# ZikangYuan/sr_livo

Measured on AMD Instinct MI355X. Metric: sweeps/s (full ESIKF solve of a 64k-pt Livox sweep vs 1M-pt voxel map), higher is better.
Workload: dtype f64; 1 GPU; HEADLINE: stream of 4 distinct 65536-keypoint livox sweeps (own poses and priors), 978481-pt voxel map (1000000 target), max_num_residuals=2147483647, r=1, K=20; one full ESIKF solve per sweep, every sweep crosses PCIe once (uploaded on the copy stream during the solve before it: resident in HBM when its solve starts); sweeps drawn with seeds 20251309 + 100 j, keeping those that take sweep 0's 2 E; parallelism=single GPU

## Files before the change

### include/srlivo_hip_debug.h

```cpp
#ifndef SRLIVO_HIP_DEBUG_H
#define SRLIVO_HIP_DEBUG_H

#include "srlivo_hip.h"

#ifdef __cplusplus
extern "C" {
#endif

int srl_debug_set_select_mode(srl_ctx *ctx, int select_mode);

int srl_debug_radix_sort_pairs(srl_ctx *ctx, const uint32_t *keys, int n, int bits, uint32_t *keys_sorted, uint32_t *positions_sorted);

int srl_debug_color_map_rebuilds(srl_ctx *ctx, int32_t *voxel_table, int32_t *grid_table);

int srl_debug_set_frame_order_mode(srl_ctx *ctx, int mode);
int srl_debug_frame_order_used(srl_ctx *ctx, int *used);

int srl_debug_set_gather_counts(srl_ctx *ctx, int nranks, int rank, const int64_t *counts);

int srl_debug_set_ablate(srl_ctx *ctx, int bits);
int srl_debug_set_fused_reduce(srl_ctx *ctx, int enable);
int srl_debug_set_bound_culling(srl_ctx *ctx, int enable);
int srl_debug_set_pose_box(srl_ctx *ctx, int kind);
int srl_debug_set_arm_linger(srl_ctx *ctx, double host_linger_us, double kernel_linger_us);
int srl_debug_pass_stamps(srl_ctx *ctx, int enable, long long *gpu_out, long long *host_out);
int srl_debug_frame_timing(srl_ctx *ctx, int enable, double out16[16]);
int srl_debug_set_frame_epoch(srl_ctx *ctx, int frames_to_wrap);
int srl_debug_set_launch_shape(srl_ctx *ctx, int keypoints_per_wave, int waves_per_workgroup);
int srl_debug_set_search_select_mode(srl_ctx *ctx, int select_mode);
int srl_debug_heap_topk(const double *distances, int n, int K, int32_t *out_index);
int srl_debug_device_sqrt(srl_ctx *ctx, const double *in, int n, double *out);
int srl_debug_block_times(srl_ctx *ctx, double *out, int max_blocks, int *nblocks);

#ifdef __cplusplus
}
#endif
#endif
```

### sr_livo_amd/capi.py

```python
import ctypes as C
import os
import re

import numpy as np

_HERE = os.path.dirname(os.path.abspath(__file__))
LIB_PATH = os.environ.get("SRL_LIB_PATH") or os.path.join(_HERE, "libsrlivo_hip.so")
INCLUDE_DIR = os.path.join(os.path.dirname(_HERE), "include")

SRL_OK = 0
SRL_ERR_NO_DEVICE = -1
SRL_ERR_BAD_ARG = -3
SRL_ERR_UNSUPPORTED = -4
SRL_ERR_COMM = -7
SRL_ERR_NAN_PLANARITY = -8
SRL_ERR_NOT_ENOUGH_RESIDUALS = -9
SRL_COMM_ID_BYTES = 128


SRL_PEER_HANDLE_BYTES = 64


class SrlError(RuntimeError):
    def __init__(self, status, what, detail=""):
# ... 119 lines not shown
        raise SrlError(-1, "libsrlivo_hip.so not built",
                       f"(expected {LIB_PATH}; run `python -c 'import __graft_entry__ as g; g.build()'`)")
    lib = C.CDLL(LIB_PATH)
    p = C.c_void_p
    dp = C.POINTER(C.c_double)
    sig = {
        "srl_device_count": ([C.POINTER(C.c_int)], C.c_int),
        "srl_ctx_create": ([C.c_int, C.POINTER(p)], C.c_int),
        "srl_ctx_destroy": ([p], C.c_int),
        "srl_last_error": ([p], C.c_char_p),
        "srl_status_str": ([C.c_int], C.c_char_p),
        "srl_icp_opts_default": ([C.POINTER(IcpOpts)], None),
        "srl_map_upload": ([p, p, p, p, C.c_int, C.c_int], C.c_int),
        "srl_map_insert": ([p, p, C.c_int, C.c_double, C.c_int, C.c_double, C.c_int, C.POINTER(C.c_int)], C.c_int),
        "srl_map_insert_report": ([p, p, C.c_int, C.c_double, C.c_int, C.c_double, C.c_int, C.c_double, p, p, C.POINTER(C.c_int),
                                   C.POINTER(C.c_int)], C.c_int),
        "srl_map_size": ([p, C.POINTER(C.c_int64), C.POINTER(C.c_int32)], C.c_int),
        "srl_map_download": ([p, p, p, p, C.c_int], C.c_int),
        "srl_map_remove_far": ([p, dp, C.c_double, C.POINTER(C.c_int32), C.POINTER(C.c_int64)], C.c_int),
        "srl_map_probe_checksum": ([p, p, C.c_int, C.c_int, C.c_double, C.POINTER(C.c_uint64)], C.c_int),
        "srl_color_opts_default": ([C.POINTER(ColorOpts)], None),
        "srl_color_map_create": ([p, C.POINTER(ColorOpts)], C.c_int),
        "srl_color_map_destroy": ([p], C.c_int),
        "srl_color_map_insert": ([p, p, C.c_int, C.c_double, C.c_double, p, p, C.c_int, p, C.c_int, C.POINTER(ColorTotals)], C.c_int),
        "srl_color_map_size": ([p, C.POINTER(C.c_int64), C.POINTER(C.c_int32), C.POINTER(C.c_int64), C.POINTER(C.c_int64)], C.c_int),
        "srl_color_map_download": ([p, p, p, p, C.c_int, p, p, C.c_int64], C.c_int),
        "srl_color_registered_download": ([p, C.c_int64, C.c_int, p], C.c_int),
        "srl_debug_color_map_rebuilds": ([p, C.POINTER(C.c_int32), C.POINTER(C.c_int32)], C.c_int),
        "srl_color_image_upload": ([p, p, C.c_int, C.c_int, C.c_int64], C.c_int),
        "srl_color_select_opts_default": ([C.POINTER(ColorSelectOpts)], None),
        "srl_color_map_select": ([p, C.POINTER(ColorCamera), C.c_int, C.c_int, p, C.c_int, C.POINTER(ColorSelectOpts), p, C.c_int64,
                                  C.POINTER(ColorSelectTotals)], C.c_int),
        "srl_color_map_render": ([p, C.POINTER(ColorCamera), p, C.c_int, C.c_double, C.POINTER(ColorRenderTotals)], C.c_int),
        "srl_color_map_download_rgb": ([p, p, p, p, p, p, C.c_int64], C.c_int),
        "srl_color_registered_rgb": ([p, C.c_int64, C.c_int, p, p, p, p, p], C.c_int),
        "srl_sweep_upload": ([p, p, C.c_int], C.c_int),
        "srl_sweep_shard": ([p, C.POINTER(C.c_int), C.POINTER(C.c_int), C.POINTER(C.c_int)], C.c_int),
        "srl_sweep_prefetch": ([p, p, C.c_int], C.c_int),
        "srl_sweep_swap": ([p], C.c_int),
        "srl_sweep_wait": ([p], C.c_int),
        "srl_thread_pin_to_gpu_numa": ([p, C.POINTER(C.c_int)], C.c_int),
        "srl_pinned_alloc": ([C.c_size_t, C.POINTER(p)], C.c_int),
        "srl_pinned_free": ([p], C.c_int),
        "srl_host_register": ([p, C.c_size_t], C.c_int),
        "srl_host_unregister": ([p], C.c_int),
        "srl_comm_backend_info": ([C.c_char_p, C.c_int, C.POINTER(C.c_int), C.POINTER(C.c_int)], C.c_int),
        "srl_build_residuals": ([p, C.POINTER(Frame), C.POINTER(IcpOpts), C.POINTER(NormalEq)], C.c_int),
        "srl_build_residuals_overlap": ([p, C.POINTER(Frame), C.POINTER(IcpOpts), C.POINTER(NormalEq), p, p], C.c_int),
        "srl_set_taps": ([p, C.c_int], C.c_int),
        "srl_fetch_neighbors": ([p, p, p, p], C.c_int),
        "srl_fetch_residuals": ([p, p, p, p, p, p, p], C.c_int),
        "srl_search_neighbors": ([p, p, C.c_int, C.c_int, C.c_double, C.c_int, C.c_int, p, p, p], C.c_int),
        "srl_transform_points": ([p, p, C.c_int, dp, dp, dp, dp, p], C.c_int),
        "srl_frame_upload": ([p, p, C.c_int], C.c_int),
        "srl_frame_undistort": ([p, p, p, p, C.c_int, p, C.c_int, C.c_double, C.c_int, dp, dp, p, p], C.c_int),
        "srl_frame_take": ([p, p, C.c_int], C.c_int),
        "srl_frame_subsample": ([p, p, C.c_int, C.c_double, C.POINTER(C.c_int)], C.c_int),
        "srl_frame_take_subsampled": ([p, p, C.c_int, p, p, p], C.c_int),
        "srl_frame_size": ([p, C.POINTER(C.c_int)], C.c_int),
        "srl_frame_select_keypoints": ([p, dp, dp, dp, dp, C.c_double, p, C.POINTER(C.c_int)], C.c_int),
        "srl_frame_commit_report": ([p, dp, dp, dp, dp, C.c_double, C.c_int, C.c_double, C.c_int, p, p, p, C.POINTER(C.c_int),
                                     C.POINTER(C.c_int)], C.c_int),
        "srl_frame_commit": ([p, dp, dp, dp, dp, C.c_double, C.c_int, C.c_double, C.c_int, p, C.POINTER(C.c_int)], C.c_int),
        "srl_comm_unique_id": ([p], C.c_int),
        "srl_comm_init_rank": ([p, C.c_int, C.c_int, p], C.c_int),
        "srl_comm_destroy": ([p], C.c_int),
        "srl_comm_set_library": ([C.c_char_p], C.c_int),
        "srl_comm_suspend": ([p, C.c_int], C.c_int),
        "srl_comm_info": ([p, C.POINTER(C.c_int), C.POINTER(C.c_int), C.POINTER(C.c_int), C.POINTER(C.c_int), C.POINTER(C.c_int64)], C.c_int),
        "srl_comm_set_host_callbacks": ([p, C.c_int, C.c_int, ALLREDUCE_FN, ALLGATHER_FN, p], C.c_int),
        "srl_debug_set_gather_counts": ([p, C.c_int, C.c_int, C.POINTER(C.c_int64)], C.c_int),
        "srl_peer_export": ([p, p, C.POINTER(p)], C.c_int),
        "srl_peer_attach": ([p, C.c_int, C.c_int, p, C.POINTER(p)], C.c_int),
        "srl_peer_set_deadline_ms": ([p, C.c_int], C.c_int),
        "srl_peer_stats": ([p, C.POINTER(C.c_int64), C.POINTER(C.c_int)], C.c_int),
        "srl_peer_detach": ([p], C.c_int),
        "srl_shard_range": ([C.c_int, C.c_int, C.c_int, C.POINTER(C.c_int), C.POINTER(C.c_int)], None),
        "srl_shard_budget": ([C.c_int, C.POINTER(C.c_int64), C.c_int, C.c_int, C.POINTER(C.c_int64), C.POINTER(C.c_int)], None),
        "srl_get_timing": ([p, C.POINTER(Timing)], C.c_int),
        "srl_debug_block_times": ([p, p, C.c_int, C.POINTER(C.c_int)], C.c_int),
        "srl_debug_set_ablate": ([p, C.c_int], C.c_int),
        "srl_debug_set_fused_reduce": ([p, C.c_int], C.c_int),
        "srl_debug_set_bound_culling": ([p, C.c_int], C.c_int),
        "srl_debug_set_pose_box": ([p, C.c_int], C.c_int),
        "srl_debug_set_arm_linger": ([p, C.c_double, C.c_double], C.c_int),
        "srl_debug_pass_stamps": ([p, C.c_int, p, p], C.c_int),
        "srl_debug_frame_timing": ([p, C.c_int, p], C.c_int),
        "srl_debug_set_frame_epoch": ([p, C.c_int], C.c_int),
        "srl_set_armed_launch": ([p, C.c_int], C.c_int),
        "srl_disarm": ([p], C.c_int),
        "srl_solve_end": ([p], C.c_int),
        "srl_get_arm_stats": ([p, C.POINTER(C.c_uint64)], C.c_int),
        "srl_debug_set_launch_shape": ([p, C.c_int, C.c_int], C.c_int),
        "srl_debug_set_search_select_mode": ([p, C.c_int], C.c_int),
        "srl_debug_set_select_mode": ([p, C.c_int], C.c_int),
        "srl_debug_set_frame_order_mode": ([p, C.c_int], C.c_int),
        "srl_debug_radix_sort_pairs": ([p, p, C.c_int, C.c_int, p, p], C.c_int),
        "srl_debug_frame_order_used": ([p, C.POINTER(C.c_int)], C.c_int),
        "srl_debug_heap_topk": ([p, C.c_int, C.c_int, p], C.c_int),
        "srl_debug_device_sqrt": ([p, p, C.c_int, p], C.c_int),
        "srl_set_profiling": ([p, C.c_int], C.c_int),
        "srl_set_profiling_period": ([p, C.c_int], C.c_int),
        "srl_timing_mark": ([p], C.c_int),
        "srl_lio_create": ([C.c_int, C.POINTER(p)], C.c_int),
        "srl_lio_destroy": ([p], C.c_int),
        "srl_lio_ctx": ([p], p),
        "srl_lio_last_error": ([p], C.c_char_p),
        "srl_lio_set_extrinsics": ([p, dp, dp], C.c_int),
        "srl_lio_set_laser_point_cov": ([p, C.c_double], C.c_int),
        "srl_lio_last_solve_launches": ([p, C.POINTER(C.c_int)], C.c_int),
        "srl_lio_eskf_get_state": ([p, dp], C.c_int),
        "srl_lio_eskf_set_state": ([p, dp], C.c_int),
        "srl_lio_eskf_get_cov": ([p, dp], C.c_int),
        "srl_lio_eskf_set_cov": ([p, dp], C.c_int),
        "srl_lio_eskf_set_noise": ([p, C.c_double, C.c_double, C.c_double, C.c_double], C.c_int),
        "srl_lio_eskf_init_imu": ([p, dp, dp], C.c_int),
        "srl_lio_eskf_scale_init_cov": ([p], C.c_int),
        "srl_lio_eskf_predict": ([p, C.c_double, dp, dp], C.c_int),
        "srl_lio_eskf_observe": ([p, dp], C.c_int),
        "srl_lio_add_points_to_map": ([p, p, C.c_int, C.c_double, C.c_int, C.c_double, C.c_int], C.c_int),
        "srl_lio_map_size": ([p, C.POINTER(C.c_int64)], C.c_int),
        "srl_lio_remove_points_far_from_location": ([p, dp, C.c_double], C.c_int),
        "srl_lio_set_collect_points_world": ([p, C.c_int], C.c_int),
        "srl_lio_points_world": ([p, p, C.c_int, C.POINTER(C.c_int)], C.c_int),
        "srl_lio_set_device_subsample": ([p, C.c_int], C.c_int),
        "srl_lio_set_color_map_options": ([p, C.POINTER(ColorOpts)], C.c_int),
        "srl_lio_set_color_times": ([p, C.c_double, C.c_double, C.c_int], C.c_int),
        "srl_lio_add_points_to_map_at": ([p, p, C.c_int, C.c_double, C.c_int, C.c_double, C.c_int, C.c_double, C.c_int], C.c_int),
        "srl_lio_select_points_for_projection": ([p, C.POINTER(ColorCamera), C.c_int, C.c_int, C.c_double, C.c_int, C.c_int, C.c_int, p, C.c_int,
                                                  C.POINTER(C.c_int), C.POINTER(ColorSelectTotals)], C.c_int),
        "srl_lio_color_visited": ([p, C.c_int, p, C.c_int, C.POINTER(C.c_int), C.POINTER(C.c_int)], C.c_int),
        "srl_lio_color_stored": ([p, p, C.c_int, C.POINTER(C.c_int)], C.c_int),
        "srl_lio_render_points_in_recent_voxel": ([p, C.POINTER(ColorCamera), C.c_double, C.POINTER(ColorRenderTotals)], C.c_int),
        "srl_lio_probe_checksum_of_committed_frame": ([p, C.c_int, C.c_double, C.POINTER(C.c_uint64), C.POINTER(C.c_int32)], C.c_int),
        "srl_lio_resident_sweep": ([p, p, C.c_int], C.c_int),
        "srl_lio_prefetch_sweep": ([p, p, C.c_int], C.c_int),
        "srl_lio_swap_sweep": ([p], C.c_int),
        "srl_lio_prefetch_sweep_during_solve": ([p, p, C.c_int], C.c_int),
        "srl_lio_update_iekf": ([p, C.POINTER(IcpOpts), p, C.c_int, dp, dp, C.c_int, p, C.c_int,
                                 C.POINTER(C.c_int), C.POINTER(C.c_int)], C.c_int),
        "srl_lio_stream_step": ([p, C.POINTER(IcpOpts), dp, dp, C.c_int, dp, dp, C.c_int, p, C.c_int, C.POINTER(C.c_int), C.POINTER(C.c_int)], C.c_int),
        "srl_lio_update_iekf_provided": ([p, C.POINTER(IcpOpts), PROVIDER_FN, p, C.c_int, dp, dp, C.c_int, p, C.c_int,
                                          C.POINTER(C.c_int), C.POINTER(C.c_int)], C.c_int),
        "srl_lio_optimize": ([p, C.POINTER(IcpOpts), C.c_double, p, p, C.c_int, dp, dp, C.c_int, p,
                              C.POINTER(C.c_int), C.POINTER(C.c_int), C.POINTER(C.c_int)], C.c_int),
        "srl_lio_eskf_try_init": ([p, dp, dp, dp, C.c_int, C.POINTER(C.c_int)], C.c_int),
        "srl_lio_eskf_get_init_stats": ([p, dp], C.c_int),
        "srl_lio_set_initial_flag": ([p, C.c_int], C.c_int),
        "srl_lio_state_initialization": ([p, C.c_int, C.c_int, dp, dp, dp], C.c_int),
        "srl_lio_set_odometry_options": ([p, C.POINTER(OdometryOpts)], C.c_int),
        "srl_lio_run_measurement": ([p, C.c_double, p, p, p, C.c_int, p, p, C.c_int, C.c_double, C.c_double,
                                     C.POINTER(ReplayResult)], C.c_int),
        "srl_lio_last_frame": ([p, C.c_int, p, p, p, C.POINTER(C.c_int)], C.c_int),
        "srl_lio_optimize_resident": ([p, C.POINTER(IcpOpts), C.c_double, p, C.c_int, dp, dp, C.c_int, p,
                                       C.POINTER(C.c_int), C.POINTER(C.c_int), C.POINTER(C.c_int)], C.c_int),
        "srl_lio_commit_frame": ([p, dp, C.c_double, C.c_int, C.c_double, C.c_int, p, C.POINTER(C.c_int)], C.c_int),
        "srl_lio_search_neighbors": ([p, dp, C.c_int, C.c_double, C.c_int, C.c_int, p, p, C.POINTER(C.c_int)], C.c_int),
        "srl_lio_neighborhood": ([p, p, C.c_int, dp, dp, dp, dp], C.c_int),
        "srl_lio_build_plane_residuals": ([p, C.POINTER(IcpOpts), p, C.c_int, dp, dp, C.c_int, p, C.c_int,
                                           C.POINTER(C.c_int), dp, C.POINTER(C.c_int), p], C.c_int),
        "srl_grid_sampling": ([p, C.c_int, C.c_double, p, C.POINTER(C.c_int)], C.c_int),
        "srl_debug_tr1_order": ([p, C.c_int, p], C.c_int),
        "srl_debug_tr1_order_by_relation": ([p, C.c_int, p], C.c_int),
    }
    for name, (argtypes, restype) in sig.items():
        fn = getattr(lib, name)
# ... 339 lines not shown
        self._chk(self.lib.srl_sweep_wait(self.h), "srl_sweep_wait")

    def sweep_swap(self):
        self._chk(self.lib.srl_sweep_swap(self.h), "srl_sweep_swap")

    def sweep_shard(self):
        b, c, t = C.c_int(), C.c_int(), C.c_int()
        self._chk(self.lib.srl_sweep_shard(self.h, C.byref(b), C.byref(c), C.byref(t)), "srl_sweep_shard")
        return b.value, c.value, t.value

    def set_taps(self, on):
        self._chk(self.lib.srl_set_taps(self.h, int(on)), "srl_set_taps")

    def set_profiling(self, on):
        self._chk(self.lib.srl_set_profiling(self.h, int(on)), "srl_set_profiling")

    def timing_mark(self):
        self._chk(self.lib.srl_timing_mark(self.h), "srl_timing_mark")

    def set_profiling_period(self, period):
        self._chk(self.lib.srl_set_profiling_period(self.h, int(period)), "srl_set_profiling_period")

    def timing(self):
        t = Timing()
        self._chk(self.lib.srl_get_timing(self.h, C.byref(t)), "srl_get_timing")
        return t

    def _select(self, opts):
        mode = int(getattr(opts, "select_mode", 0) or 0)
        if mode != getattr(self, "_select_mode", 0):
            self._chk(self.lib.srl_debug_set_select_mode(self.h, mode), "srl_debug_set_select_mode")
            self._select_mode = mode

    def build_residuals(self, frame, opts, allow=(SRL_ERR_NAN_PLANARITY,)):
        self._select(opts)
        out = NormalEq()
        rc = self._chk(self.lib.srl_build_residuals(self.h, C.byref(frame), C.byref(opts), C.byref(out)), "srl_build_residuals", ok=allow)
        return out, rc

    def build_residuals_overlap(self, frame, opts, fn, allow=(SRL_ERR_NAN_PLANARITY,)):
        self._select(opts)
        out = NormalEq()
        cb = C.CFUNCTYPE(None, C.c_void_p)(lambda _u: fn())
        rc = self._chk(self.lib.srl_build_residuals_overlap(self.h, C.byref(frame), C.byref(opts), C.byref(out), cb, None),
                       "srl_build_residuals_overlap", ok=allow)
        return out, rc

    def pin_thread_to_gpu_numa(self):
        node = C.c_int(-1)
        rc = self.lib.srl_thread_pin_to_gpu_numa(self.h, C.byref(node))
        return node.value if rc == 0 else None

    def fetch_neighbors(self, K=20):
        _, n, _ = self.sweep_shard()
        ids = np.empty((n, K), dtype=np.int32)
        status = np.empty(n, dtype=np.uint8)
        ncand = np.empty(n, dtype=np.int32)
        self._chk(self.lib.srl_fetch_neighbors(self.h, _ptr(ids), _ptr(status), _ptr(ncand)), "srl_fetch_neighbors")
        return ids, status, ncand

    def fetch_residuals(self):
        _, n, _ = self.sweep_shard()
        normal = np.empty((n, 3)); a2d = np.empty(n); w = np.empty(n); off = np.empty(n); d = np.empty(n); J = np.empty((n, 6))
        self._chk(self.lib.srl_fetch_residuals(self.h, _ptr(normal), _ptr(a2d), _ptr(w), _ptr(off), _ptr(d), _ptr(J)), "srl_fetch_residuals")
        return dict(normal=normal, a2D=a2d, weight=w, norm_offset=off, distance=d, jacobian=J)

    def search_neighbors(self, world_xyz, nb=1, size=1.0, K=20, thr=1):
        q = _f64(world_xyz, (-1, 3))
        ids = np.empty((len(q), K), dtype=np.int32)
        xyz = np.empty((len(q), K, 3), dtype=np.float32)
        nf = np.empty(len(q), dtype=np.int32)
        self._chk(self.lib.srl_search_neighbors(self.h, _ptr(q), len(q), nb, size, K, thr, _ptr(ids), _ptr(xyz), _ptr(nf)), "srl_search_neighbors")
        return ids, xyz, nf

    def set_launch_shape(self, kpw, wpb):
        self._chk(self.lib.srl_debug_set_launch_shape(self.h, int(kpw), int(wpb)), "srl_debug_set_launch_shape")

    def set_fused_reduce(self, on):
        self._chk(self.lib.srl_debug_set_fused_reduce(self.h, 1 if on else 0), "srl_debug_set_fused_reduce")

    def set_bound_culling(self, on):
        self._chk(self.lib.srl_debug_set_bound_culling(self.h, 1 if on else 0), "srl_debug_set_bound_culling")

    def set_search_select_mode(self, mode):
        self._chk(self.lib.srl_debug_set_search_select_mode(self.h, int(mode)), "srl_debug_set_search_select_mode")

    def set_armed_launch(self, on):
        mode = int(on) if on in (0, 1, 2) and not isinstance(on, bool) else (1 if on else 0)
        self._chk(self.lib.srl_set_armed_launch(self.h, mode), "srl_set_armed_launch")

    def solve_end(self):
        self._chk(self.lib.srl_solve_end(self.h), "srl_solve_end")

    def disarm(self):
        self._chk(self.lib.srl_disarm(self.h), "srl_disarm")

    def arm_stats(self):
        out = (C.c_uint64 * 4)()
        self._chk(self.lib.srl_get_arm_stats(self.h, out), "srl_get_arm_stats")
        return dict(zip(("armed", "fired", "cancelled", "expired"), (int(v) for v in out)))

    def set_pose_box(self, kind):
        self._chk(self.lib.srl_debug_set_pose_box(self.h, int(kind)), "srl_debug_set_pose_box")

    FRAME_STAGES = ("upload", "select_group", "select_download", "select_host_order", "select_gather", "commit_transform", "commit_download",
                    "insert_sort", "insert_segments", "insert_lookup_create", "insert_replay")

    def set_frame_epoch(self, frames_to_wrap):
        self._chk(self.lib.srl_debug_set_frame_epoch(self.h, int(frames_to_wrap)), "srl_debug_set_frame_epoch")

    def frame_timing(self, enable=True):
        out = np.zeros(16)
        self._chk(self.lib.srl_debug_frame_timing(self.h, 1 if enable else 0, _ptr(out)), "srl_debug_frame_timing")
        return dict(zip(self.FRAME_STAGES, (float(v) for v in out)))

    def pass_stamps(self, enable=True, read=True):
        g = np.zeros((64, 32), dtype=np.int64); h = np.zeros((64, 4), dtype=np.int64)
        self._chk(self.lib.srl_debug_pass_stamps(self.h, 1 if enable else 0, _ptr(g) if read else None, _ptr(h) if read else None), "srl_debug_pass_stamps")
        return g, h

    def set_arm_linger(self, host_linger_us=150.0, kernel_linger_us=300.0):
        self._chk(self.lib.srl_debug_set_arm_linger(self.h, float(host_linger_us), float(kernel_linger_us)), "srl_debug_set_arm_linger")

    def device_sqrt(self, x):
        x = _f64(x).ravel()
        out = np.empty_like(x)
        self._chk(self.lib.srl_debug_device_sqrt(self.h, _ptr(x), len(x), _ptr(out)), "srl_debug_device_sqrt")
        return out

    def transform_points(self, raw_xyz, q, t, R_il=None, t_il=None):
        r = _f64(raw_xyz, (-1, 3))
        out = np.empty_like(r)
        R_il = _f64(np.eye(3) if R_il is None else R_il).ravel()
        t_il = _f64(np.zeros(3) if t_il is None else t_il)
        self._chk(self.lib.srl_transform_points(self.h, _ptr(r), len(r), _dptr(_f64(q)), _dptr(_f64(t)), _dptr(R_il), _dptr(t_il), _ptr(out)), "srl_transform_points")
        return out

    def frame_upload(self, raw_xyz):
        r = _f64(raw_xyz, (-1, 3))
        self._chk(self.lib.srl_frame_upload(self.h, _ptr(r), len(r)), "srl_frame_upload")

    def frame_undistort(self, raw_xyz, relative_time_ms, imu_states, time_frame_begin, mode, R_il=None, t_il=None, imu_point_in=None,
                        want_outputs=True):
        r = _f64(raw_xyz, (-1, 3)); rel = _f64(relative_time_ms)
        st = _f64(imu_states, (-1, 17))
        R_il = _f64(np.eye(3) if R_il is None else R_il).ravel()
        t_il = _f64(np.zeros(3) if t_il is None else t_il)
        pin = None if imu_point_in is None else _f64(imu_point_in, (-1, 3))
        imu = np.empty_like(r) if want_outputs else None
        out = np.empty_like(r) if want_outputs else None
        self._chk(self.lib.srl_frame_undistort(self.h, _ptr(r), _ptr(rel), None if pin is None else _ptr(pin), len(r), _ptr(st), len(st),
                                               float(time_frame_begin), int(mode), _dptr(R_il), _dptr(t_il), _ptr(imu), _ptr(out)),
                  "srl_frame_undistort")
        return imu, out

    def frame_take(self, index):
        idx = np.ascontiguousarray(index, dtype=np.int32)
        self._chk(self.lib.srl_frame_take(self.h, _ptr(idx), len(idx)), "srl_frame_take")

    def frame_subsample(self, order, sample_size):
        o = np.ascontiguousarray(order, dtype=np.int32)
        m = C.c_int()
        self._chk(self.lib.srl_frame_subsample(self.h, _ptr(o), len(o), float(sample_size), C.byref(m)), "srl_frame_subsample")
        self._kept = m.value
        return m.value

# ... 494 lines not shown
```

### sr_livo_amd/csrc/srl_capi.cpp

```cpp
#include "../../include/srlivo_hip.h"
#include "../../include/srlivo_hip_debug.h"
#include "host/srl_la.h"
#include "srl_device.h"
#include "srl_hash.h"
#include "srl_heap.h"

#include <hip/hip_runtime.h>
#include <sched.h>

#include <algorithm>
#include <atomic>
#include <chrono>
#include <climits>
#include <cstdio>
#include <cstdlib>
#include <cstring>
#include <mutex>
#include <string>
#include <vector>

struct SrlMapState;
int srl_map_insert_device(struct srl_ctx *ctx, const double *world_xyz, int n, double voxel_size, int cap,
                          double min_distance_points, int min_num_points, int *num_added);

#include "srl_ctx.h"
int srl_map_insert_report_device(srl_ctx *ctx, const double *world_xyz, int n, double voxel_size, int cap, double min_distance_points, int min_num_points,
                                 double ref_z, uint8_t *outcome, srl_cloud_point *cloud, int *num_cloud, int *num_added);

namespace {

unsigned next_pow2(unsigned v) { unsigned p = 1; while (p < v) p <<= 1; return p; }
inline long long steady_ns() { return std::chrono::duration_cast<std::chrono::nanoseconds>(std::chrono::steady_clock::now().time_since_epoch()).count(); }

constexpr int SRL_MAX_DEVICES = 64;
std::atomic<int> g_live_ctx[SRL_MAX_DEVICES];
inline int live_contexts(int device) { return (device >= 0 && device < SRL_MAX_DEVICES) ? g_live_ctx[device].load(std::memory_order_relaxed) : 1; }

int ensure_work(srl_ctx *ctx, int n) {
    if (n <= ctx->work_cap) return SRL_OK;
    const int cap = std::max(n, 1024);
    const int nblocks = std::max((cap + SRL_KPB - 1) / SRL_KPB, 1024 + 8);
    int rc;
    if ((rc = ensure(ctx, ctx->d_rec, (size_t)cap * 8))) return rc;
    if ((rc = ensure(ctx, ctx->d_status, (size_t)cap))) return rc;
    if ((rc = ensure(ctx, ctx->d_bound, (size_t)cap * 4))) return rc;
    ctx->bound_n = 0;
    if ((rc = ensure(ctx, ctx->d_partials, (size_t)nblocks * SRL_PART_STRIDE))) return rc;
    if ((rc = ensure(ctx, ctx->d_binfo, (size_t)nblocks))) return rc;
    ctx->work_cap = cap;
    ctx->block_cap = nblocks;
    return SRL_OK;
}

bool srl_is_pinned(const void *p) {
    hipPointerAttribute_t attr;
    if (hipPointerGetAttributes(&attr, p) != hipSuccess) { (void)hipGetLastError(); return false; }
    return attr.type == hipMemoryTypeHost;
}

int srl_ring_init(srl_ctx *ctx) {
    if (ctx->h_ring) return SRL_OK;
    HIPCHK(ctx, hipHostMalloc((void **)&ctx->h_ring, (size_t)srl_ctx::RING_SLOTS * srl_ctx::RING_SLOT_BYTES, hipHostMallocDefault));
    for (int i = 0; i < srl_ctx::RING_SLOTS; i++) { HIPCHK(ctx, hipEventCreateWithFlags(&ctx->ring_ev[i], hipEventDisableTiming)); ctx->ring_busy[i] = false; }
    return SRL_OK;
}

int ensure_taps(srl_ctx *ctx, int n, int K) {
    if (n <= ctx->tap_cap && K <= ctx->tap_K) return SRL_OK;
    const int cap = std::max(n, ctx->tap_cap), kk = std::max(K, ctx->tap_K);
    int rc;
    if ((rc = ensure(ctx, ctx->d_tap_ids, (size_t)cap * kk))) return rc;
    if ((rc = ensure(ctx, ctx->d_tap_ncand, (size_t)cap))) return rc;
    if ((rc = ensure(ctx, ctx->d_tap_normal, (size_t)cap * 3))) return rc;
    if ((rc = ensure(ctx, ctx->d_tap_a2d, (size_t)cap))) return rc;
    if ((rc = ensure(ctx, ctx->d_tap_offset, (size_t)cap))) return rc;
    ctx->tap_cap = cap;
    ctx->tap_K = kk;
    return SRL_OK;
}

}

int srl_ctx_ensure_work(srl_ctx *ctx, int n) { return ensure_work(ctx, n); }
bool srl_ctx_is_pinned(const void *p) { return srl_is_pinned(p); }

int srl_ctx_grow_map(srl_ctx *ctx, unsigned need_slabs, unsigned need_slots);

extern "C" {

int srl_device_count(int *count) {
    int c = 0;
    if (hipGetDeviceCount(&c) != hipSuccess) { if (count) *count = 0; return SRL_ERR_NO_DEVICE; }
    if (count) *count = c;
    return SRL_OK;
}

const char *srl_status_str(int s) {
    switch (s) {
        case SRL_OK: return "ok";
        case SRL_ERR_NO_DEVICE: return "no HIP device (the product has no CPU fallback)";
        case SRL_ERR_HIP: return "HIP runtime error";
        case SRL_ERR_BAD_ARG: return "bad argument";
        case SRL_ERR_UNSUPPORTED: return "option outside the supported envelope";
        case SRL_ERR_NO_MAP: return "no map uploaded";
        case SRL_ERR_NO_SWEEP: return "no sweep uploaded";
        case SRL_ERR_COMM: return "RCCL error";
        case SRL_ERR_NAN_PLANARITY: return "NaN planarity (optimize.cpp:348-350 throws)";
        case SRL_ERR_NOT_ENOUGH_RESIDUALS: return "not enough residuals (optimize.cpp:110)";
        default: return "unknown status";
    }
}

void srl_icp_opts_default(srl_icp_opts *o) {
    o->threshold_voxel_occupancy = 1;
    o->init_num_frames = 20;
    o->size_voxel_map = 1.0;
    o->num_iters_icp = 5;
    o->min_number_neighbors = 20;
    o->voxel_neighborhood = 1;
    o->power_planarity = 2.0;
    o->max_number_neighbors = 20;
    o->max_dist_to_plane_icp = 0.3;
    o->threshold_orientation_norm = 0.1;
    o->threshold_translation_norm = 0.01;
    o->max_num_residuals = 600;
    o->weight_alpha = 0.9;
    o->weight_neighborhood = 0.1;
}

int srl_ctx_create(int device, srl_ctx **out) {
    if (!out) return SRL_ERR_BAD_ARG;
    *out = nullptr;
    int count = 0;
    if (hipGetDeviceCount(&count) != hipSuccess || count <= 0 || device < 0 || device >= count) return SRL_ERR_NO_DEVICE;
    if (hipSetDevice(device) != hipSuccess) return SRL_ERR_NO_DEVICE;
    srl_ctx *ctx = new srl_ctx();
    ctx->device = device;
    { int cu = 0; if (hipDeviceGetAttribute(&cu, hipDeviceAttributeMultiprocessorCount, device) == hipSuccess && cu > 0) ctx->num_cu = cu; }
    if (hipStreamCreateWithFlags(&ctx->stream, hipStreamNonBlocking) != hipSuccess) { delete ctx; return SRL_ERR_NO_DEVICE; }
    if (hipMalloc((void **)&ctx->d_out, sizeof(SrlDevOut)) != hipSuccess ||
        hipHostMalloc((void **)&ctx->h_out, sizeof(SrlDevOut)) != hipSuccess ||
        hipMalloc((void **)&ctx->d_count, sizeof(long long)) != hipSuccess ||
        hipHostMalloc((void **)&ctx->h_count, sizeof(long long)) != hipSuccess) {
        delete ctx;
        return SRL_ERR_HIP;
    }
    {
        const size_t row_bytes = (size_t)(SRL_FUSED_MAX_BLOCKS + SRL_FUSED_MAX_GROUPS) * SRL_ROW_GRANULES * 8;
        if (hipMalloc((void **)&ctx->d_granules, row_bytes) != hipSuccess || hipMemset(ctx->d_granules, 0, row_bytes) != hipSuccess) { delete ctx; return SRL_ERR_HIP; }
    }
    if (hipHostMalloc((void **)&ctx->h_mail, sizeof(SrlMailbox), hipHostMallocCoherent | hipHostMallocMapped) != hipSuccess) {
        delete ctx;
        return SRL_ERR_HIP;
    }
    std::memset(ctx->h_mail, 0, sizeof(SrlMailbox));
    for (int i = 0; i < 4; i++) hipEventCreate(&ctx->ev[i]);
    if (device < SRL_MAX_DEVICES) g_live_ctx[device].fetch_add(1, std::memory_order_relaxed);
    ctx->counted = true;
    *out = ctx;
    return SRL_OK;
}

int srl_ctx_destroy(srl_ctx *ctx) {
    if (!ctx) return SRL_OK;
    hipSetDevice(ctx->device);
    if (ctx->counted && ctx->device < SRL_MAX_DEVICES) g_live_ctx[ctx->device].fetch_sub(1, std::memory_order_relaxed);
    if (ctx->armed) srl_ctx_disarm(ctx);
    if (ctx->stream) hipStreamSynchronize(ctx->stream);
    if (ctx->copy_stream) hipStreamSynchronize(ctx->copy_stream);
    if (ctx->color) srl_color_map_destroy(ctx);
    if (ctx->pose_box_pinned) hipHostFree(ctx->pose_box_pinned);
    if (ctx->pose_box_dev) hipFree(ctx->pose_box_dev);
    if (ctx->d_pose_relay) hipFree(ctx->d_pose_relay);
    if (ctx->comm && srl_rccl()) srl_rccl()->CommDestroy(ctx->comm);
    if (ctx->parked_comm && srl_rccl()) srl_rccl()->CommDestroy(ctx->parked_comm);
    if (ctx->d_sub_kept) hipFree(ctx->d_sub_kept);
    if (ctx->d_sub_seen) hipFree(ctx->d_sub_seen);
    void *bufs[] = {ctx->d_corr_in, ctx->d_corr_rel, ctx->d_corr_imu, ctx->d_corr_raw, ctx->d_corr_seg, ctx->d_frame_raw, ctx->d_frame_world, ctx->d_table, ctx->d_slabs, ctx->d_raw, ctx->d_rec, ctx->d_status, ctx->d_partials, ctx->d_binfo,
                    ctx->d_out, ctx->d_count, ctx->d_bound, ctx->d_granules, ctx->d_rec_granules, ctx->d_raw_next, ctx->d_stage_next, ctx->d_stage_cur, ctx->d_tap_ids, ctx->d_tap_ncand, ctx->d_tap_normal, ctx->d_tap_a2d,
                    ctx->d_tap_offset, ctx->d_gather, ctx->d_peer, ctx->d_mail};
    for (int r = 0; r < SRL_MAX_PEERS; r++) if (ctx->peer_mapped[r]) hipIpcCloseMemHandle(ctx->peer_mapped[r]);
    if (ctx->d_inbox) hipFree(ctx->d_inbox);
    for (void *b : bufs) if (b) hipFree(b);
    if (ctx->h_out) hipHostFree(ctx->h_out);
    if (ctx->h_count) hipHostFree(ctx->h_count);
    if (ctx->h_mail) hipHostFree(ctx->h_mail);
    if (ctx->h_arm_stamps) hipHostFree(ctx->h_arm_stamps);
    if (ctx->h_scratch) hipHostFree(ctx->h_scratch);
    if (ctx->h_frame_x) hipHostFree(ctx->h_frame_x);
    for (SrlEpochTable *t : {&ctx->sel_table, &ctx->ins_table}) { if (t->keyw) hipFree(t->keyw); if (t->minw) hipFree(t->minw); }
    if (ctx->d_frame_sync) hipFree(ctx->d_frame_sync);
    if (ctx->d_tr1_sched) hipFree(ctx->d_tr1_sched);
    if (ctx->h_insert_cnt) hipHostFree(ctx->h_insert_cnt);
    if (ctx->ev_insert) hipEventDestroy(ctx->ev_insert);
    if (ctx->ev_world) hipEventDestroy(ctx->ev_world);
    if (ctx->ev_frame_read) hipEventDestroy(ctx->ev_frame_read);
    if (ctx->h_ring) { hipHostFree(ctx->h_ring); for (int i = 0; i < srl_ctx::RING_SLOTS; i++) if (ctx->ring_ev[i]) hipEventDestroy(ctx->ring_ev[i]); }
    for (auto &b : ctx->pool_free) hipFree(b.p);
    ctx->pool_free.clear();
    for (int i = 0; i < 4; i++) if (ctx->ev[i]) hipEventDestroy(ctx->ev[i]);
    for (int i = 0; i < srl_ctx::PROF_RING; i++) for (int k = 0; k < 2; k++) if (ctx->ring[i][k]) hipEventDestroy(ctx->ring[i][k]);
    for (int sl = 0; sl < 2; sl++) for (int k = 0; k < 2; k++) if (ctx->up_ev[sl][k]) hipEventDestroy(ctx->up_ev[sl][k]);
    if (ctx->upload_ev) hipEventDestroy(ctx->upload_ev);
    if (ctx->copy_stream) { hipStreamSynchronize(ctx->copy_stream); hipStreamDestroy(ctx->copy_stream); }
    if (ctx->prefix_stream) { hipStreamSynchronize(ctx->prefix_stream); hipStreamDestroy(ctx->prefix_stream); }
    if (ctx->stream) hipStreamDestroy(ctx->stream);
    delete ctx;
    return SRL_OK;
}

const char *srl_last_error(const srl_ctx *ctx) { return ctx ? ctx->err.c_str() : "null context"; }

int srl_map_upload(srl_ctx *ctx, const int16_t *keys_xyz, const int32_t *counts, const float *xyz, int V, int cap) {
    if (!ctx || V < 0 || (V > 0 && (!keys_xyz || !counts || !xyz))) return SRL_ERR_BAD_ARG;
    SRL_DISARM(ctx);
    if (cap != SRL_VOXEL_CAP) { ctx->err = "max_num_points_in_voxel must be 20"; return SRL_ERR_UNSUPPORTED; }
    HIPCHK(ctx, hipSetDevice(ctx->device));
    { const int rcs = srl_map_settle(ctx); if (rcs) return rcs; }
    ctx->bound_n = 0;
    const unsigned slab_cap = std::max<unsigned>(1024u, (unsigned)V + (unsigned)V / 2u + 4096u);
    if (slab_cap > SRL_MAX_SLABS) { ctx->err = "map too large: slab byte offsets are 32-bit (16.7 M voxels)"; return SRL_ERR_UNSUPPORTED; }
    const unsigned table_cap = next_pow2(std::max<unsigned>(2048u, SRL_TABLE_FACTOR * slab_cap));
    std::vector<SrlSlab> slabs((size_t)V);
    std::vector<SrlMapSlot> table((size_t)table_cap);
    for (auto &s : table) { s.key = SRL_EMPTY_KEY; s.slab = 0; s.count = 0; }
    long long npts = 0;
    const unsigned mask = table_cap - 1;
    for (int v = 0; v < V; v++) {
        SrlSlab &s = slabs[v];
        std::memset(&s, 0, sizeof s);
        const int c = counts[v];
        if (c < 0 || c > cap) { ctx->err = "voxel count out of range"; return SRL_ERR_BAD_ARG; }
        for (int i = 0; i < c; i++)
            for (int d = 0; d < 3; d++) s.xyz[i][d] = xyz[((size_t)v * cap + i) * 3 + d];
        s.count = (unsigned)c;
        s.key = srl_pack_key(keys_xyz[3 * v], keys_xyz[3 * v + 1], keys_xyz[3 * v + 2]);
        npts += c;
        unsigned h = srl_hash_key(s.key) & mask;
        while (table[h].key != SRL_EMPTY_KEY) {
            if (table[h].key == s.key) { ctx->err = "duplicate voxel key in upload"; return SRL_ERR_BAD_ARG; }
            h = (h + 1) & mask;
        }
        table[h].key = s.key;
        table[h].slab = (unsigned)v;
        table[h].count = (unsigned)c;
    }
    if (ctx->d_slabs) { HIPCHK(ctx, hipFree(ctx->d_slabs)); ctx->d_slabs = nullptr; }
    if (ctx->d_table) { HIPCHK(ctx, hipFree(ctx->d_table)); ctx->d_table = nullptr; }
    HIPCHK(ctx, hipMalloc((void **)&ctx->d_slabs, ((size_t)slab_cap + 1) * SRL_SLAB_BYTES));
    HIPCHK(ctx, hipMemsetD32Async((hipDeviceptr_t)(ctx->d_slabs + (size_t)slab_cap * SRL_SLAB_BYTES), 0x7f800000, SRL_SLAB_BYTES / 4, ctx->stream));
    HIPCHK(ctx, hipMalloc((void **)&ctx->d_table, (size_t)table_cap * sizeof(SrlMapSlot)));
    HIPCHK(ctx, hipMemsetAsync(ctx->d_slabs, 0, (size_t)slab_cap * SRL_SLAB_BYTES, ctx->stream));
    if (V > 0) HIPCHK(ctx, hipMemcpyAsync(ctx->d_slabs, slabs.data(), (size_t)V * SRL_SLAB_BYTES, hipMemcpyHostToDevice, ctx->stream));
    HIPCHK(ctx, hipMemcpyAsync(ctx->d_table, table.data(), (size_t)table_cap * sizeof(SrlMapSlot), hipMemcpyHostToDevice, ctx->stream));
    HIPCHK(ctx, hipStreamSynchronize(ctx->stream));
    ctx->slab_cap = slab_cap;
    ctx->table_cap = table_cap;
    ctx->num_voxels = V;
    ctx->num_points = npts;
    return SRL_OK;
}

// ... 567 lines not shown
    if (ctx->force_kpw) {
        p.kpw = ctx->force_kpw;
        const bool only16 = p.kpw != 4 && p.kpw != 8 && p.kpw != 16;
        p.wpb = ((ctx->force_wpb == 16 || only16) && srl_assoc_lds_bytes(p.K, p.nb, p.kpw, 16) <= SRL_LDS_LIMIT) ? 16 : 4;
        if (only16 && p.wpb != 16) p.kpw = 4;
    }
    if (ctx->ablate != 0 && srl_assoc_lds_bytes(p.K, p.nb, 16, 16) <= SRL_LDS_LIMIT) { p.kpw = 16; p.wpb = 16; }
    p.kpb = p.kpw * p.wpb;
    p.nblocks = (n_eff + p.kpb - 1) / p.kpb;

    p.cut = cut_possible(ctx, o);
    p.transport = pass_transport(ctx);
    p.dbg_gather = ctx->dbg_gather;
    const bool fusable = !ctx->taps && ctx->ablate == 0 && o->max_num_residuals > 0 && ctx->fuse_reduce && !ctx->dbg_gather;
    p.fuse_cut = fusable && p.cut && p.transport == Transport::single && p.wpb == 16 && p.kpb <= SRL_FUSED_CUT_MAX_KPB && p.nblocks <= 512;
    p.fused = p.fuse_cut || (fusable && !p.cut && p.wpb == 16 && p.nblocks <= SRL_FUSED_MAX_BLOCKS);
    p.tagged_mail = p.fused && p.transport != Transport::rccl;
    p.mailbox = p.transport != Transport::rccl && (p.transport == Transport::single || p.fused);
    const bool fast_sel = ctx->select_mode == 0 || ctx->select_mode == 4;
    p.arm_ok = ctx->arm_mode != 0 && p.fused && fast_sel && ctx->profiling != 1 && (p.transport != Transport::host_callback || ctx->cb_ar);
    return SRL_OK;
}

static void prepare_assoc_args(srl_ctx *ctx, const srl_frame *f, const srl_icp_opts *o, int n_eff, const PassPlan &p, SrlAssocArgs &a) {
    std::memset(&a, 0, sizeof a);
    a.raw_x = ctx->d_raw;
    a.raw_y = ctx->d_raw + ctx->sweep_cap;
    a.raw_z = ctx->d_raw + 2 * (size_t)ctx->sweep_cap;
    a.n = n_eff;
    a.aos = (n_eff > ctx->soa_valid_n) ? ctx->d_stage_cur : nullptr;
    a.table = ctx->d_table;
    a.table_mask = ctx->table_cap - 1;
    a.slabs = ctx->d_slabs;
    a.inf_off = ctx->slab_cap * (unsigned)SRL_SLAB_BYTES;
    a.write_rec = ((ctx->taps || p.cut) && !p.fuse_cut) ? 1 : 0;
    {
        const srl::Quat q(f->q[0], f->q[1], f->q[2], f->q[3]);
        const srl::Mat3 Rn = q.normalized().toRotationMatrix();
        const srl::Mat3 R = q.toRotationMatrix();
        std::memcpy(a.Rn, Rn.a, sizeof a.Rn);
        std::memcpy(a.R, R.a, sizeof a.R);
    }
    std::memcpy(a.t, f->t, sizeof a.t);
    std::memcpy(a.t_last, f->t_last, sizeof a.t_last);
    std::memcpy(a.R_il, f->R_il, sizeof a.R_il);
    std::memcpy(a.t_il, f->t_il, sizeof a.t_il);
    a.size_voxel = o->size_voxel_map;
    a.max_dist = o->max_dist_to_plane_icp;
    {
        double lw = std::abs(o->weight_alpha), ln = std::abs(o->weight_neighborhood);
        const double sum = lw + ln;
        lw /= sum;
        ln /= sum;
        a.lambda_w = lw;
        a.lambda_n = ln;
    }
    a.power_planarity = o->power_planarity;
    a.nbr_scale = o->max_dist_to_plane_icp * o->min_number_neighbors;
    a.K = p.K;
    a.min_nb = o->min_number_neighbors;
    a.thr_cap = p.thr;
    a.select_mode = ctx->select_mode;
    a.ablate = ctx->ablate;
    a.stamps = ctx->h_arm_stamps;
    a.rec = ctx->d_rec;
    a.status = ctx->d_status;
    a.partials = ctx->d_partials;
    a.binfo = ctx->d_binfo;
    if (ctx->taps) {
        a.tap_ids = ctx->d_tap_ids;
        a.tap_ncand = ctx->d_tap_ncand;
        a.tap_normal = ctx->d_tap_normal;
        a.tap_a2d = ctx->d_tap_a2d;
        a.tap_offset = ctx->d_tap_offset;
    }
    {
        float sv = (float)o->size_voxel_map;
        int sv_bits; std::memcpy(&sv_bits, &sv, 4);
        const int sig[4] = {p.K, p.nb, p.thr, sv_bits};
        if (std::memcmp(sig, ctx->bound_sig, sizeof sig) != 0) { ctx->bound_n = 0; std::memcpy(ctx->bound_sig, sig, sizeof sig); }
        a.bound_out = ctx->d_bound;
        a.bound_in = ctx->bound_mode != 0 ? ctx->d_bound : nullptr;
        a.bound_use = a.bound_in ? std::min(ctx->bound_n, n_eff) : 0;
    }
    if (p.fused) {
        a.granules = ctx->d_granules;
        a.mailbox = p.transport == Transport::rccl ? ctx->d_mail : ctx->h_mail;
        a.mail_tagged = p.tagged_mail ? 1 : 0;
    }
    if (p.fuse_cut) {
        a.rec_granules = ctx->d_rec_granules;
        a.cut_max = o->max_num_residuals;
    }
}

static int grow_pass_buffers(srl_ctx *ctx, const PassPlan &p) {
    int rc;
    ctx->taps_valid = false;
    if (ctx->taps) {
        if ((rc = ensure_taps(ctx, ctx->n, p.K))) return rc;
        if (ctx->n > 0) {
            HIPCHK(ctx, hipMemsetAsync(ctx->d_tap_ids, 0xFF, (size_t)ctx->n * p.K * sizeof(int), ctx->stream));
            HIPCHK(ctx, hipMemsetAsync(ctx->d_tap_normal, 0, (size_t)ctx->n * 3 * sizeof(double), ctx->stream));
            HIPCHK(ctx, hipMemsetAsync(ctx->d_tap_a2d, 0, (size_t)ctx->n * sizeof(double), ctx->stream));
            HIPCHK(ctx, hipMemsetAsync(ctx->d_tap_offset, 0, (size_t)ctx->n * sizeof(double), ctx->stream));
        }
    }
    ctx->last_nblocks = p.nblocks;
    if (p.nblocks > ctx->block_cap) {
        if ((rc = ensure(ctx, ctx->d_partials, (size_t)p.nblocks * SRL_PART_STRIDE))) return rc;
        if ((rc = ensure(ctx, ctx->d_binfo, (size_t)p.nblocks))) return rc;
        ctx->block_cap = p.nblocks;
    }
    if (ctx->profiling == 2 && ctx->ring_head - ctx->ring_tail >= (unsigned)srl_ctx::PROF_RING && (rc = drain_ring(ctx, true))) return rc;
    if (p.fused && p.transport == Transport::rccl && !ctx->d_mail && (rc = ensure(ctx, ctx->d_mail, 1))) return rc;
    const size_t need = (size_t)p.nblocks * p.kpb * 16;
    if (p.fuse_cut && need > ctx->rec_granule_cap) {
        if ((rc = ensure(ctx, ctx->d_rec_granules, need))) return rc;
        HIPCHK(ctx, hipMemsetAsync(ctx->d_rec_granules, 0, need * sizeof(unsigned long long), ctx->stream));
        ctx->rec_granule_cap = need;
    }
    return SRL_OK;
}

struct ExchangeTag { unsigned long long seq; unsigned epoch; int slot; };
static ExchangeTag exchange_tag(unsigned long long seq) {
    if ((unsigned)seq == 0u) ++seq;
    return {seq, (unsigned)seq, (int)(seq & 1ull)};
}
static ExchangeTag next_exchange(srl_ctx *ctx) {
    const ExchangeTag t = exchange_tag(ctx->peer_seq + 1);
    ctx->peer_seq = t.seq;
    return t;
}

static SrlAssocArgs arm_signature(const SrlAssocArgs &src) {
    SrlAssocArgs sg = src;
    std::memset(sg.Rn, 0, sizeof sg.Rn); std::memset(sg.R, 0, sizeof sg.R); std::memset(sg.t, 0, sizeof sg.t);
    std::memset(sg.t_last, 0, sizeof sg.t_last);
    sg.pose_box = nullptr; sg.pose_relay = nullptr; sg.pose_relayed = 0; sg.pose_epoch = 0; sg.arm_linger_ticks = 0;
    sg.raw_x = sg.raw_y = sg.raw_z = nullptr; sg.alt_x = sg.alt_y = sg.alt_z = nullptr; sg.n = 0; sg.aos = nullptr; sg.alt_aos = nullptr;
    sg.bound_use = 0;
    return sg;
}

static int fire_or_cancel(srl_ctx *ctx, const PassPlan &p, SrlAssocArgs &a, unsigned long long &seq_now, bool &fired) {
    fired = false;
    bool needs_tail = false;
    if (ctx->tail_pending) {
        if (hipEventQuery(ctx->up_ev[ctx->cur_slot][1]) == hipSuccess) { ctx->tail_pending = false; ctx->cur_prefix_n = ctx->n; }
        else needs_tail = a.n > ctx->cur_prefix_n;
        (void)hipGetLastError();
    }
    if (!ctx->armed) return SRL_OK;
    const SrlAssocArgs sg = arm_signature(a);
    const double age_us = (double)(steady_ns() - ctx->armed_at_ns) * 1e-3;
    const bool on_raw = a.raw_x == ctx->armed_raw && ctx->sweep_cap == ctx->armed_raw_cap && a.aos == nullptr;
    const bool on_alt = !on_raw && ctx->armed_alt != nullptr && a.raw_x == ctx->armed_alt && ctx->sweep_cap == ctx->armed_alt_cap &&
                        a.aos != nullptr && a.aos == ctx->armed_alt_aos;
    if (p.arm_ok && !needs_tail && age_us < ctx->arm_host_linger_us && p.nb == ctx->armed_nb && p.kpw == ctx->armed_kpw &&
        p.nblocks <= ctx->armed_nblocks && (on_raw || on_alt) && std::memcmp(&sg, &ctx->armed_sig, sizeof sg) == 0) {
        pose_box_write(ctx, a.Rn, a.R, a.t, (unsigned)seq_now, SRL_ARM_GO | (on_alt ? SRL_ARM_ALT : 0u), (unsigned)a.n, a.t_last);
        ctx->armed = false;
        ctx->armed_ring = -1;
        ctx->arm_stats[1]++;
        ctx->cur_measured = ctx->armed_measured;
        ctx->cur_gen = ctx->armed_gen;
        fired = true;
        return SRL_OK;
    }
    if (const int rc = srl_ctx_disarm(ctx)) return rc;
    seq_now = ++ctx->seq;
    if (p.fused) a.seq = seq_now;
    return SRL_OK;
}

static int prof_role(const srl_ctx *ctx) {
    if (ctx->prof_period <= 1) return 2;
    const unsigned long long r = ctx->prof_count % (unsigned long long)ctx->prof_period;
    return r == 1 ? 2 : (r == 0 ? 1 : 0);
}

static int launch_assoc(srl_ctx *ctx, const PassPlan &p, const SrlAssocArgs &args, bool armed) {
    if (!armed && ctx->tail_pending) {
        HIPCHK(ctx, hipStreamWaitEvent(ctx->stream, ctx->up_ev[ctx->cur_slot][1], 0));
        ctx->tail_pending = false; ctx->cur_prefix_n = ctx->n;
    }
    const bool prof = ctx->profiling == 1, prof_light = ctx->profiling == 2;
    const int role = prof_light ? prof_role(ctx) : 0;
    int prev = -1;
    if (armed && role != 0) {
        int rc;
        if (ctx->ring_head - ctx->ring_tail >= (unsigned)srl_ctx::PROF_RING - 2 && (rc = drain_ring(ctx, true))) return rc;
        if (ctx->ring_head != 0 && !ctx->ring_void[(ctx->ring_head - 1) % srl_ctx::PROF_RING] && ctx->ring_last_count == (long long)ctx->prof_count - 1)
            prev = (int)((ctx->ring_head - 1) % srl_ctx::PROF_RING);
    }
    const unsigned slot = ctx->ring_head % srl_ctx::PROF_RING;
    if (prof) HIPCHK(ctx, hipEventRecord(ctx->ev[0], ctx->stream));
    if (role == 2 && prev < 0) HIPCHK(ctx, hipEventRecord(ctx->ring[slot][0], ctx->stream));
    HIPCHK(ctx, srl_launch_assoc(args, p.nb, p.kpw, p.wpb, ctx->stream));
    if (prof) HIPCHK(ctx, hipEventRecord(ctx->ev[1], ctx->stream));
    if (role != 0) {
        HIPCHK(ctx, hipEventRecord(ctx->ring[slot][1], ctx->stream));
        ctx->ring_prev[slot] = prev; ctx->ring_marker[slot] = role == 1; ctx->ring_void[slot] = false; ctx->ring_gen[slot] = ctx->timing_gen;
        ctx->ring_last_count = (long long)ctx->prof_count;
        ctx->ring_head++;
    }
    if (prof_light) ctx->prof_count++;
    const bool measured = !prof_light || role == 2;
    if (armed) { ctx->armed_ring = role != 0 ? (int)slot : -1; ctx->armed_measured = measured; ctx->armed_gen = ctx->timing_gen; }
    else { ctx->cur_measured = measured; ctx->cur_gen = ctx->timing_gen; }
    return SRL_OK;
}

static bool arm_wanted(const srl_ctx *ctx) {
    return ctx->arm_mode == 2 ||
           (live_contexts(ctx->device) <= 1 && !ctx->peer_shares_device && !ctx->comm_shares_device &&
            (ctx->next_n >= 0 || ctx->expected_passes == 0 || ctx->passes_in_solve + 1 < ctx->expected_passes));
}

static int arm_next(srl_ctx *ctx, const PassPlan &p, const SrlAssocArgs &a) {
    int rc;
    if ((rc = ensure_pose_box(ctx))) return rc;
    SrlAssocArgs nx = a;
    nx.seq = ctx->seq + 1;
    nx.bound_use = a.bound_in ? a.n : 0;
    const bool has_alt = ctx->d_raw_next != nullptr && ctx->next_cap > 0 && ctx->d_stage_next != nullptr;
    nx.aos = nullptr;
    nx.alt_aos = has_alt ? ctx->d_stage_next : nullptr;
    nx.alt_x = has_alt ? ctx->d_raw_next : nullptr;
    nx.alt_y = has_alt ? ctx->d_raw_next + ctx->next_cap : nullptr;
    nx.alt_z = has_alt ? ctx->d_raw_next + 2 * (size_t)ctx->next_cap : nullptr;
    if (p.transport == Transport::peer) {
        const ExchangeTag t = exchange_tag(ctx->peer_seq + 1);
        nx.peer_epoch = t.epoch;
        nx.peer_slot = t.slot;
    }
    nx.pose_box = ctx->h_pose_box;
    nx.pose_relay = ctx->d_pose_relay;
    nx.pose_relayed = ctx->pose_box_kind == 1 ? 0 : 1;
    nx.pose_epoch = (unsigned)nx.seq;
    nx.arm_linger_ticks = ctx->arm_linger_ticks;
    if ((rc = launch_assoc(ctx, p, nx, true))) return rc;
    ctx->armed_sig = arm_signature(nx);
    ctx->armed_nb = p.nb; ctx->armed_kpw = p.kpw; ctx->armed_nblocks = p.nblocks;
    ctx->armed_raw = nx.raw_x; ctx->armed_raw_cap = ctx->sweep_cap;
    ctx->armed_alt = nx.alt_x; ctx->armed_alt_cap = has_alt ? ctx->next_cap : 0; ctx->armed_alt_aos = nx.alt_aos;
    ctx->armed_at_ns = steady_ns();
    ctx->armed = true;
    ctx->arm_stats[0]++;
    return SRL_OK;
}

static int reduce_unfused(srl_ctx *ctx, const PassPlan &p, const srl_icp_opts *o, int n_eff, unsigned long long seq) {
    int64_t budget = o->max_num_residuals;
    int mode = 0;
    const long long *gather = nullptr;
    if (p.transport == Transport::single || !p.cut) {
        srl_shard_budget(o->max_num_residuals, nullptr, ctx->nranks, ctx->rank, &budget, &mode);
    } else {
        HIPCHK(ctx, srl_launch_count(ctx->d_binfo, p.nblocks, o->max_num_residuals <= 0 ? 1 : 0, ctx->d_count, ctx->stream));
        if (p.transport == Transport::peer) {
            const ExchangeTag t = next_exchange(ctx);
            HIPCHK(ctx, srl_launch_peer_counts(ctx->d_peer, t.epoch, t.slot, ctx->d_count, ctx->d_gather, ctx->stream));
            gather = ctx->d_gather;
        } else if (p.transport == Transport::rccl) {
            NCCLCHK(ctx, AllGather(ctx->d_count, ctx->d_gather, 1, ncclInt64, ctx->comm, ctx->stream));
            gather = ctx->d_gather;
        } else if (p.dbg_gather) {
            gather = ctx->d_gather;
        } else {
            HIPCHK(ctx, hipMemcpyAsync(ctx->h_count, ctx->d_count, sizeof(long long), hipMemcpyDeviceToHost, ctx->stream));
            HIPCHK(ctx, hipStreamSynchronize(ctx->stream));
            if (!ctx->cb_ag) { ctx->err = "nranks > 1 without communicator"; return SRL_ERR_COMM; }
            int64_t mine = *ctx->h_count;
            std::vector<int64_t> all64((size_t)ctx->nranks, 0);
            if (ctx->cb_ag(&mine, all64.data(), ctx->cb_user) != 0) { ctx->err = "allgather callback failed"; return SRL_ERR_COMM; }
            srl_shard_budget(o->max_num_residuals, all64.data(), ctx->nranks, ctx->rank, &budget, &mode);
        }
    }
    SrlReduceArgs ra;
    ra.rec = ctx->d_rec;
    ra.status = ctx->d_status;
    ra.partials = ctx->d_partials;
    ra.binfo = ctx->d_binfo;
    ra.n = n_eff;
    ra.kpb = p.kpb;
    ra.nblocks = p.nblocks;
    ra.max_res = budget;
    ra.gather = gather;
    ra.rank = ctx->rank;
    ra.max_num_residuals = o->max_num_residuals;
    ra.out = ctx->d_out;
    ra.mailbox = p.mailbox ? ctx->h_mail : nullptr;
    ra.seq = seq;
    HIPCHK(ctx, srl_launch_reduce(ra, mode, ctx->stream));
    if (p.transport == Transport::peer) {
        const ExchangeTag t = next_exchange(ctx);
        HIPCHK(ctx, srl_launch_peer_rows(ctx->d_peer, t.epoch, t.slot, ctx->d_out, ctx->h_mail, seq, gather, ctx->stream));
    }
    return SRL_OK;
}

static int host_allreduce(srl_ctx *ctx, SrlDevOut *out) {
    if (!ctx->cb_ar) { ctx->err = "nranks > 1 without communicator"; return SRL_ERR_COMM; }
    if (ctx->cb_ar(reinterpret_cast<double *>(out), SRL_REDUCED_DOUBLES, ctx->cb_user) != 0) { ctx->err = "allreduce callback failed"; return SRL_ERR_COMM; }
    return SRL_OK;
}

// ... 14 lines not shown
            ctx->arm_stats[3]++;
            ctx->err = "armed launch expired";
            return SRL_INTERNAL_ARM_EXPIRED;
        }
        if ((++spins & 0xFFFFF) == 0) {
            const hipError_t qe = hipStreamQuery(ctx->stream);
            if (qe != hipSuccess && qe != hipErrorNotReady) { ctx->err = std::string("reduce kernel: ") + hipGetErrorString(qe); return SRL_ERR_HIP; }
            if (qe == hipSuccess && !mail_arrived(ctx, p.tagged_mail, seq)) {
                const unsigned long long *gran = ctx->h_mail->g;
                char dbg[256];
                int bad = -1; unsigned bad_tag = 0;
                if (p.tagged_mail) for (int i = 0; i < 2 * OUT_WORDS; i++) if ((unsigned)(gran[i] >> 32) != (unsigned)seq) { bad = i; bad_tag = (unsigned)(gran[i] >> 32); break; }
                std::snprintf(dbg, sizeof dbg, "reduce kernel finished without publishing (seq %llu, tagged %d, fired %d, fused %d, blocks %d, first stale granule %d tag %u, plain seq %llu)",
                              seq, (int)p.tagged_mail, (int)fired, (int)p.fused, p.nblocks, bad, bad_tag, (unsigned long long)ctx->h_mail->seq);
                ctx->err = dbg;
                return SRL_ERR_HIP;
            }
        }
    }
    if (p.tagged_mail) {
        const unsigned long long *gran = ctx->h_mail->g;
        unsigned long long *w = reinterpret_cast<unsigned long long *>(ctx->h_out);
        for (int i = 0; i < OUT_WORDS; i++)
            w[i] = (__atomic_load_n(&gran[2 * i], __ATOMIC_RELAXED) & 0xFFFFFFFFull) | (__atomic_load_n(&gran[2 * i + 1], __ATOMIC_RELAXED) << 32);
    } else {
        std::memcpy(ctx->h_out, &ctx->h_mail->out, sizeof(SrlDevOut));
    }
    return SRL_OK;
}

static int wait_result(srl_ctx *ctx, const PassPlan &p, unsigned long long seq, bool fired, long long &last_visited_local) {
    const bool copied = p.transport == Transport::host_callback && !p.fused;
    int rc;
    if (copied) {
        HIPCHK(ctx, hipMemcpyAsync(ctx->h_out, ctx->d_out, sizeof(SrlDevOut), hipMemcpyDeviceToHost, ctx->stream));
        HIPCHK(ctx, hipStreamSynchronize(ctx->stream));
    } else if ((rc = read_mailbox(ctx, p, seq, fired))) {
        return rc;
    }
    last_visited_local = ctx->h_out->last_visited;
    if (p.transport == Transport::host_callback && (rc = host_allreduce(ctx, ctx->h_out))) return rc;
    if (copied) {
        if (ctx->h_out->d_timeout > 0.5) { ctx->err = "fused final reduction timed out on another rank"; return SRL_INTERNAL_FUSED_TIMEOUT; }
        return SRL_OK;
    }
    if (ctx->h_out->pad == SRL_PEER_TIMEOUT_MARK) {
        ctx->err = "direct peer exchange: a rank's row has not arrived yet";
        return SRL_INTERNAL_PEER_TIMEOUT;
    }
    if (ctx->h_out->pad != 0 || ctx->h_out->d_timeout > 0.5) {
        ctx->err = "fused final reduction timed out waiting for a workgroup's row";
        if (fired && p.transport == Transport::rccl) ctx->arm_stats[3]++;
        return SRL_INTERNAL_FUSED_TIMEOUT;
    }
    return SRL_OK;
}

static int finish_pass(srl_ctx *ctx, const PassPlan &p, const srl_icp_opts *o, const SrlAssocArgs &a, int n_eff, long long last_visited_local,
                       unsigned long long seq, bool fired, srl_normal_eq *out) {
    const SrlDevOut &r = *ctx->h_out;
    const long long visited_total = (long long)(r.d_visited + 0.5);
    if (p.fused && !p.fuse_cut) {
        const long long expect = ctx->nranks > 1 ? (long long)ctx->total_n : (long long)n_eff;
        if (visited_total != expect) {
            char buf[256];
            std::snprintf(buf, sizeof buf, "fused pass visited %lld of %lld keypoints (fired %d, seq %llu; residuals %.0f, time-out flag %.0f, marker %lld)", visited_total, expect,
                          (int)fired, seq, r.d_num_res, r.d_timeout, (long long)r.pad);
            ctx->err = buf;
            return SRL_ERR_HIP;
        }
    }
    std::memcpy(out->HtH, r.HtH, sizeof out->HtH);
    std::memcpy(out->Hth, r.Hth, sizeof out->Hth);
    out->loss_sum = r.loss;
    out->num_residuals = (int32_t)(r.d_num_res + 0.5);
    out->success = out->num_residuals >= o->min_number_neighbors ? 1 : 0;
    out->sum_candidates = (int64_t)(r.d_sum_pk + 0.5);
    out->last_visited = visited_total - 1;
    out->nan_error = r.d_nan > 0.5 ? 1 : 0;
    out->num_fallback = (int32_t)(r.d_fallback + 0.5);

    if (a.aos != nullptr && n_eff > ctx->soa_valid_n) ctx->soa_valid_n = n_eff;
    ctx->bound_n = n_eff;
    ctx->last_K = p.K;
    ctx->last_nb = p.nb;
    ctx->last_visited_local = last_visited_local;
    ctx->taps_valid = ctx->taps;
    return SRL_OK;
}

struct PassClock { std::chrono::steady_clock::time_point entry, prep, launched, enq, res; };

static long long clock_ns(std::chrono::steady_clock::time_point t) {
    return std::chrono::duration_cast<std::chrono::nanoseconds>(t.time_since_epoch()).count();
}

static int account_pass(srl_ctx *ctx, const PassPlan &p, int n_eff, const PassClock &c) {
    using us = std::chrono::duration<double, std::micro>;
    using ms = std::chrono::duration<double, std::milli>;
    const bool prof = ctx->profiling == 1, prof_light = ctx->profiling == 2;
    if (prof) {
        HIPCHK(ctx, hipEventSynchronize(ctx->ev[3]));
        hipEventElapsedTime(&ctx->timing.assoc_ms, ctx->ev[0], ctx->ev[1]);
        hipEventElapsedTime(&ctx->timing.reduce_ms, ctx->ev[1], ctx->ev[2]);
        hipEventElapsedTime(&ctx->timing.total_ms, ctx->ev[0], ctx->ev[3]);
        ctx->timing.calls += 1;
        ctx->timing.sum_assoc_ms += ctx->timing.assoc_ms;
        ctx->timing.sum_reduce_ms += ctx->timing.reduce_ms;
        ctx->timing.sum_total_ms += ctx->timing.total_ms;
        ctx->timing.sum_keypoints += n_eff;
        const auto t_end = std::chrono::steady_clock::now();
        ctx->timing.sum_host_launch_us += us(c.enq - c.entry).count();
        ctx->timing.sum_host_wait_us += us(c.res - c.enq).count();
        ctx->timing.sum_host_total_us += us(t_end - c.entry).count();
    }
    const double sum_pk = ctx->h_out->d_sum_pk;
    const long long side = 2 * p.nb + 1;
    const long long per_kp = 24 + 12 * side * side * side;
    const double pk_share = (ctx->nranks > 1 && ctx->total_n > 0) ? sum_pk * ((double)ctx->n / (double)ctx->total_n) : sum_pk;
    ctx->timing.algorithmic_bytes = per_kp * (long long)n_eff + (long long)(12.0 * pk_share);
    if (prof || (prof_light && ctx->cur_measured && ctx->cur_gen == ctx->timing_gen)) {
        ctx->timing.sum_algorithmic_bytes += ctx->timing.algorithmic_bytes; ctx->timing.sum_keypoints += prof_light ? n_eff : 0; ctx->timing.sum_passes += 1;
    }
    if (ctx->profiling == 3) {
        ctx->timing.calls += 1;
        ctx->timing.sum_host_launch_us += us(c.launched - c.prep).count();
        ctx->timing.sum_host_wait_us += us(c.res - c.enq).count();
        ctx->timing.sum_host_total_us += us(std::chrono::steady_clock::now() - c.entry).count();
        ctx->timing.sum_assoc_ms += ms(c.prep - c.entry).count();
        ctx->timing.sum_reduce_ms += ms(c.enq - c.launched).count();
    }
    return SRL_OK;
}

static int build_residuals_pass(srl_ctx *ctx, const srl_frame *f, const srl_icp_opts *o, srl_normal_eq *out, int n_eff) {
    PassClock clk{std::chrono::steady_clock::now()};
    HIPCHK(ctx, hipSetDevice(ctx->device));
    PassPlan p;
    int rc;
    if ((rc = plan_pass(ctx, f, o, n_eff, p))) return rc;
    if ((rc = grow_pass_buffers(ctx, p))) return rc;
    SrlAssocArgs a;
    prepare_assoc_args(ctx, f, o, n_eff, p, a);
    unsigned long long seq_now = ++ctx->seq;
    if (p.transport == Transport::peer && ctx->peer_failed) {
        ctx->err = "direct peer exchange: this session has failed (a rank's row never arrived); srl_peer_detach, srl_peer_export and srl_peer_attach on every rank start a new one";
        return SRL_ERR_COMM;
    }
    if (p.fused) a.seq = seq_now;
    if (p.fused && p.transport == Transport::peer) {
        const ExchangeTag t = next_exchange(ctx);
        a.peer = ctx->d_peer; a.peer_epoch = t.epoch; a.peer_slot = t.slot;
    }
    bool fired = false;
    if ((rc = fire_or_cancel(ctx, p, a, seq_now, fired))) return rc;
    clk.prep = std::chrono::steady_clock::now();
    if (!fired && (rc = launch_assoc(ctx, p, a, false))) return rc;
    clk.launched = std::chrono::steady_clock::now();
    long long *stamps = ctx->h_arm_stamps ? ctx->arm_host_stamps[seq_now & 63ull] : nullptr;
    if (stamps) { stamps[0] = clock_ns(clk.entry); stamps[1] = clock_ns(clk.launched); stamps[3] = fired ? 1 : 0; }
    const bool arm = p.arm_ok && arm_wanted(ctx);
    if (arm && p.transport != Transport::rccl && (rc = arm_next(ctx, p, a))) return rc;
    if (!p.fused && (rc = reduce_unfused(ctx, p, o, n_eff, seq_now))) return rc;
    if (ctx->profiling == 1) HIPCHK(ctx, hipEventRecord(ctx->ev[2], ctx->stream));
    clk.enq = std::chrono::steady_clock::now();
    if (ctx->overlap_fn) {
// ... 53 lines not shown
        if (distance) distance[k] = rec[(size_t)k * 8 + 6];
        if (weight) weight[k] = rec[(size_t)k * 8 + 7];
    }
    return SRL_OK;
}

int srl_search_neighbors(srl_ctx *ctx, const double *world_xyz, int n, int nb_voxels_visited, double size_voxel_map,
                         int max_num_neighbors, int threshold_voxel_capacity, int32_t *ids, float *nb_xyz,
                         int32_t *num_found) {
    if (!ctx || n < 0 || (n > 0 && (!world_xyz || !ids || !num_found))) return SRL_ERR_BAD_ARG;
    SRL_DISARM(ctx);
    if (!ctx->d_table) return SRL_ERR_NO_MAP;
    if (nb_voxels_visited < 1 || nb_voxels_visited > 2) { ctx->err = "nb_voxels_visited must be 1 or 2"; return SRL_ERR_UNSUPPORTED; }
    if (max_num_neighbors < 1 || max_num_neighbors > SRL_MAX_NEIGHBORS) { ctx->err = "max_num_neighbors must be in [1,32]"; return SRL_ERR_UNSUPPORTED; }
    if (n == 0) return SRL_OK;
    HIPCHK(ctx, hipSetDevice(ctx->device));
    const int K = max_num_neighbors;
    DevBuf b_q, b_ids, b_nf, b_xyz;
    HIPCHK(ctx, b_q.alloc(ctx, (size_t)n * 3 * sizeof(double)));
    HIPCHK(ctx, b_ids.alloc(ctx, (size_t)n * K * sizeof(int)));
    HIPCHK(ctx, b_nf.alloc(ctx, (size_t)n * sizeof(int)));
    if (nb_xyz) HIPCHK(ctx, b_xyz.alloc(ctx, (size_t)n * K * 3 * sizeof(float)));
    double *d_q = b_q.as<double>();
    int *d_ids = b_ids.as<int>(), *d_nf = b_nf.as<int>();
    float *d_xyz = nb_xyz ? b_xyz.as<float>() : nullptr;
    HIPCHK(ctx, hipMemcpyAsync(d_q, world_xyz, (size_t)n * 3 * sizeof(double), hipMemcpyHostToDevice, ctx->stream));
    HIPCHK(ctx, hipMemsetAsync(d_ids, 0xFF, (size_t)n * K * sizeof(int), ctx->stream));
    if (d_xyz) HIPCHK(ctx, hipMemsetAsync(d_xyz, 0, (size_t)n * K * 3 * sizeof(float), ctx->stream));
    SrlSearchArgs a;
    a.q = d_q; a.n = n; a.table = ctx->d_table; a.table_mask = ctx->table_cap - 1; a.slabs = ctx->d_slabs;
    a.size_voxel = size_voxel_map; a.K = K; a.thr_cap = threshold_voxel_capacity; a.select_mode = ctx->search_select_mode;
    a.ids = d_ids; a.nb_xyz = d_xyz; a.num_found = d_nf;
    HIPCHK(ctx, srl_launch_search(a, nb_voxels_visited, ctx->stream));
    HIPCHK(ctx, hipMemcpyAsync(ids, d_ids, (size_t)n * K * sizeof(int), hipMemcpyDeviceToHost, ctx->stream));
    HIPCHK(ctx, hipMemcpyAsync(num_found, d_nf, (size_t)n * sizeof(int), hipMemcpyDeviceToHost, ctx->stream));
    if (nb_xyz) HIPCHK(ctx, hipMemcpyAsync(nb_xyz, d_xyz, (size_t)n * K * 3 * sizeof(float), hipMemcpyDeviceToHost, ctx->stream));
    HIPCHK(ctx, hipStreamSynchronize(ctx->stream));
    return SRL_OK;
}

int srl_transform_points(srl_ctx *ctx, const double *raw_xyz, int n, const double q[4], const double t[3],
                         const double R_il[9], const double t_il[3], double *out_xyz) {
    if (!ctx || n < 0 || (n > 0 && (!raw_xyz || !out_xyz)) || !q || !t || !R_il || !t_il) return SRL_ERR_BAD_ARG;
    SRL_DISARM(ctx);
    if (n == 0) return SRL_OK;
    HIPCHK(ctx, hipSetDevice(ctx->device));
    DevBuf b_in, b_o;
    HIPCHK(ctx, b_in.alloc(ctx, (size_t)n * 3 * sizeof(double)));
    HIPCHK(ctx, b_o.alloc(ctx, (size_t)n * 3 * sizeof(double)));
    double *d_in = b_in.as<double>(), *d_o = b_o.as<double>();
    HIPCHK(ctx, hipMemcpyAsync(d_in, raw_xyz, (size_t)n * 3 * sizeof(double), hipMemcpyHostToDevice, ctx->stream));
    SrlXform X;
    const srl::Mat3 R = srl::Quat(q[0], q[1], q[2], q[3]).toRotationMatrix();
    std::memcpy(X.R, R.a, sizeof X.R);
    std::memcpy(X.t, t, sizeof X.t);
    std::memcpy(X.R_il, R_il, sizeof X.R_il);
    std::memcpy(X.t_il, t_il, sizeof X.t_il);
    HIPCHK(ctx, srl_launch_transform(d_in, n, X, d_o, ctx->stream));
    HIPCHK(ctx, hipMemcpyAsync(out_xyz, d_o, (size_t)n * 3 * sizeof(double), hipMemcpyDeviceToHost, ctx->stream));
    HIPCHK(ctx, hipStreamSynchronize(ctx->stream));
    return SRL_OK;
}

int srl_debug_set_ablate(srl_ctx *ctx, int bits) {
    if (!ctx) return SRL_ERR_BAD_ARG;
    SRL_DISARM(ctx);
    ctx->ablate = bits;
    return SRL_OK;
}
int srl_debug_set_launch_shape(srl_ctx *ctx, int keypoints_per_wave, int waves_per_workgroup) {
    if (!ctx) return SRL_ERR_BAD_ARG;
    SRL_DISARM(ctx);
    if (keypoints_per_wave != 0 && keypoints_per_wave != 2 && keypoints_per_wave != 3 && keypoints_per_wave != 6 && keypoints_per_wave != 12 && keypoints_per_wave != 4 && keypoints_per_wave != 8 && keypoints_per_wave != 16) return SRL_ERR_BAD_ARG;
    if (waves_per_workgroup != 0 && waves_per_workgroup != 4 && waves_per_workgroup != 16) return SRL_ERR_BAD_ARG;
    ctx->force_kpw = keypoints_per_wave;
    ctx->force_wpb = waves_per_workgroup;
    return SRL_OK;
}
int srl_debug_set_bound_culling(srl_ctx *ctx, int enable) {
    if (!ctx) return SRL_ERR_BAD_ARG;
    SRL_DISARM(ctx);
    ctx->bound_mode = enable ? 1 : 0;
    ctx->bound_n = 0;
    return SRL_OK;
}
int srl_debug_set_fused_reduce(srl_ctx *ctx, int enable) {
    if (!ctx) return SRL_ERR_BAD_ARG;
    SRL_DISARM(ctx);
    ctx->fuse_reduce = enable != 0;
    return SRL_OK;
}
int srl_debug_set_select_mode(srl_ctx *ctx, int select_mode) {
    if (!ctx || select_mode < 0 || select_mode > 5) return SRL_ERR_BAD_ARG;
    SRL_DISARM(ctx);
    ctx->select_mode = select_mode;
    return SRL_OK;
}
int srl_debug_set_frame_order_mode(srl_ctx *ctx, int mode) {
    if (!ctx || mode < 0 || mode > 1) return SRL_ERR_BAD_ARG;
    ctx->frame_order_mode = mode;
    return SRL_OK;
}
int srl_debug_frame_order_used(srl_ctx *ctx, int *used) {
    if (!ctx || !used) return SRL_ERR_BAD_ARG;
    *used = ctx->frame_order_used;
    return SRL_OK;
}
int srl_debug_set_search_select_mode(srl_ctx *ctx, int select_mode) {
    if (!ctx || select_mode < 0 || select_mode > 5) return SRL_ERR_BAD_ARG;
    ctx->search_select_mode = select_mode;
    return SRL_OK;
}
int srl_debug_heap_topk(const double *distances, int n, int K, int32_t *out_index) {
    if (n < 0 || K < 1 || K > SRL_MAX_NEIGHBORS || (n > 0 && !distances) || !out_index) return SRL_ERR_BAD_ARG;
    double hd[SRL_MAX_NEIGHBORS];
    int he[SRL_MAX_NEIGHBORS];
    int size = 0;
    for (int i = 0; i < n; i++) size = srl_heap_offer(hd, he, size, K, distances[i], i);
    int out[SRL_MAX_NEIGHBORS];
    srl_heap_drain(hd, he, size, out);
    for (int i = 0; i < size; i++) out_index[i] = out[i];
    return size;
}
int srl_debug_device_sqrt(srl_ctx *ctx, const double *in, int n, double *out) {
    if (!ctx || n < 0 || (n > 0 && (!in || !out))) return SRL_ERR_BAD_ARG;
    SRL_DISARM(ctx);
    if (n == 0) return SRL_OK;
    HIPCHK(ctx, hipSetDevice(ctx->device));
    DevBuf b;
    HIPCHK(ctx, b.alloc(ctx, (size_t)n * sizeof(double)));
    HIPCHK(ctx, hipMemcpyAsync(b.as<double>(), in, (size_t)n * sizeof(double), hipMemcpyHostToDevice, ctx->stream));
    HIPCHK(ctx, srl_launch_sqrt(b.as<double>(), n, ctx->stream));
    HIPCHK(ctx, hipMemcpyAsync(out, b.as<double>(), (size_t)n * sizeof(double), hipMemcpyDeviceToHost, ctx->stream));
    HIPCHK(ctx, hipStreamSynchronize(ctx->stream));
    return SRL_OK;
}

void srl_shard_range(int n, int nranks, int rank, int *begin, int *count) {
    const long long b = (long long)rank * n / nranks;
    const long long e = (long long)(rank + 1) * n / nranks;
    if (begin) *begin = (int)b;
    if (count) *count = (int)(e - b);
}

void srl_shard_budget(int max_num_residuals, const int64_t *accepted_per_rank, int nranks, int rank,
                      int64_t *budget, int *mode) {
    (void)nranks;
    int64_t b = max_num_residuals;
    int m = 0;
    if (max_num_residuals <= 0) {
        int64_t prior = 0;
        for (int r = 0; r < rank; r++) prior += accepted_per_rank ? accepted_per_rank[r] : (int64_t)1;
        m = (prior > 0) ? 2 : 1;
    } else {
        int64_t prior = 0;
        for (int r = 0; r < rank; r++) prior += accepted_per_rank ? accepted_per_rank[r] : 0;
        b = (int64_t)max_num_residuals - prior;
        if (b <= 0) m = 2;
    }
    if (budget) *budget = b;
    if (mode) *mode = m;
}

int srl_build_residuals(srl_ctx *ctx, const srl_frame *f, const srl_icp_opts *o, srl_normal_eq *out) {
    if (!ctx || !f || !o || !out) return SRL_ERR_BAD_ARG;
    if (!ctx->d_table) return SRL_ERR_NO_MAP;
// ... 331 lines not shown
```

### sr_livo_amd/csrc/srl_ctx.h

```cpp
#pragma once
#include "../../include/srlivo_hip.h"
#include "srl_device.h"
#include "host/tr1_relation.h"

#include <hip/hip_runtime.h>
#include "srl_rccl.h"

#include <string>
#include <vector>

struct SrlEpochTable {
    unsigned long long *keyw = nullptr;
    unsigned long long *minw = nullptr;
    unsigned cap = 0;
    unsigned epoch16 = 0;
    unsigned counter32 = 0;
};

#define SRL_PEER_POISON_WORD SRL_PEER_INBOX_GRANULES
#define SRL_PEER_DEVICE_WORD (SRL_PEER_INBOX_GRANULES + 1)
#define SRL_PEER_INBOX_ALLOC_GRANULES (SRL_PEER_INBOX_GRANULES + 8)

struct srl_ctx {
    int device = 0;
    bool counted = false;
    hipStream_t stream = nullptr;
    std::string err;

    SrlMapSlot *d_table = nullptr;
    unsigned table_cap = 0;
    unsigned char *d_slabs = nullptr;
    unsigned slab_cap = 0;
    int num_voxels = 0;
    long long num_points = 0;

    double *d_raw = nullptr;
    int sweep_cap = 0;
    int n = 0;
    int shard_begin = 0;
    int total_n = 0;
    bool sweep_loaded = false;
    int search_select_mode = 0;
    int select_mode = 0;
    int ablate = 0;
    void (*overlap_fn)(void *) = nullptr;
    void *overlap_user = nullptr;

    double *d_raw_next = nullptr;
    double *d_stage_next = nullptr;
    double *d_stage_cur = nullptr;
    int soa_valid_n = 0;
    int next_cap = 0, stage_next_cap = 0, stage_cur_cap = 0;
    int next_n = -1, next_begin = 0, next_total = 0;
    hipStream_t copy_stream = nullptr;
    hipStream_t prefix_stream = nullptr;
    int num_cu = 256;
    hipEvent_t next_ready = nullptr;
    hipEvent_t up_ev[2][2] = {};
    bool up_one_dma[2] = {true, true};
    int next_slot = 0;
    int next_prefix_n = 0;
    int prefix_hint = 0;
    float *d_bound = nullptr;
    int bound_n = 0;
    int bound_sig[4] = {0, 0, 0, 0};
    int bound_mode = 1;
    bool tail_pending = false;
    int cur_slot = 0, cur_prefix_n = 0;

    double *d_frame_raw = nullptr;
    double *d_frame_world = nullptr;
    int frame_cap = 0;
    int frame_n = -1;
    int frame_world_n = -1;
    bool frame_world_seen = false;
    struct SrlColorMap *color = nullptr;
    double *d_corr_in = nullptr, *d_corr_rel = nullptr, *d_corr_imu = nullptr, *d_corr_raw = nullptr;
    int *d_corr_seg = nullptr;
    int corr_cap = 0;
    int corr_n = -1;
    int *d_sub_kept = nullptr;
    unsigned *d_sub_seen = nullptr;
    int sub_cap = 0;
    int sub_n = -1;
    unsigned sub_seen_tag = 0;

    bool frame_timing = false;
    double frame_stage_us[16] = {};
    long long frame_stage_last_ns = 0;

    hipEvent_t upload_ev = nullptr;
    bool upload_pending = false;

    static constexpr int RING_SLOTS = 4;
    static constexpr int RING_SLOT_BYTES = 256 * 1024;
    char *h_ring = nullptr;
    hipEvent_t ring_ev[RING_SLOTS] = {};
    bool ring_busy[RING_SLOTS] = {};
    unsigned ring_next = 0;

    char *h_scratch = nullptr;
    size_t h_scratch_bytes = 0;
    char *h_frame_x = nullptr;
    size_t h_frame_x_bytes = 0;
    unsigned *d_frame_sync = nullptr;
    unsigned frame_tag = 0;
    SrlTr1Sched *d_tr1_sched = nullptr;
    int tr1_steps = -1;
    unsigned tr1_first[SRL_TR1_MAX_STEPS] = {0}, tr1_nb[SRL_TR1_MAX_STEPS + 1] = {0};
    int frame_order_mode = 0;
    int frame_order_used = 0;
    int *h_insert_cnt = nullptr;
    hipEvent_t ev_insert = nullptr, ev_world = nullptr;
    bool insert_pending = false;
    hipEvent_t ev_frame_read = nullptr;
    SrlEpochTable sel_table, ins_table;

    double *d_rec = nullptr;
    unsigned char *d_status = nullptr;
    double *d_partials = nullptr;
    SrlBlockInfo *d_binfo = nullptr;
    int work_cap = 0;
    int block_cap = 0;
    SrlDevOut *d_out = nullptr;
    SrlDevOut *h_out = nullptr;
    long long *d_count = nullptr;
    long long *h_count = nullptr;
    unsigned long long *d_rec_granules = nullptr;
    size_t rec_granule_cap = 0;
    unsigned long long *d_granules = nullptr;
    int force_kpw = 0, force_wpb = 0;
    bool fuse_reduce = true;
    SrlMailbox *h_mail = nullptr;
    unsigned long long seq = 0;

    int arm_mode = 1;
    int passes_in_solve = 0;
    int expected_passes = 0;
    int pose_box_kind = -1;
    bool pose_box_dev_visible = false;
    unsigned long long *h_pose_box = nullptr;
    unsigned long long *pose_box_pinned = nullptr;
    unsigned long long *pose_box_dev = nullptr;
    unsigned long long *d_pose_relay = nullptr;
    bool armed = false;
    SrlAssocArgs armed_sig;
    int armed_nb = 0, armed_kpw = 0;
    int armed_nblocks = 0;
    const double *armed_raw = nullptr, *armed_alt = nullptr;
// ... 195 lines not shown
```

### sr_livo_amd/csrc/srl_device.h

```cpp
#pragma once
#include <hip/hip_runtime.h>
#include <stddef.h>
#include <stdint.h>


#define SRL_CAP 20
#define SRL_SLAB_BYTES 256
#define SRL_MAX_SLABS 16777215u
#ifndef SRL_KPB
#define SRL_KPB 64
#endif
#ifndef SRL_ASSOC_WAVES_PER_SIMD
#define SRL_ASSOC_WAVES_PER_SIMD 4
#endif
#define SRL_BLOCK 256
#define SRL_SURV_CAP 64
#define SRL_WAVE_SCRATCH 2048
#define SRL_MAXK 32
#define SRL_EMPTY_KEY 0xFFFFFFFFFFFFFFFFull
#define SRL_TABLE_FACTOR 4u
#define SRL_PART_STRIDE 32
#define SRL_ROW_GRANULES 128
#define SRL_FUSED_MAX_BLOCKS 2048
#define SRL_FUSED_GROUP 256
#define SRL_FUSED_MAX_GROUPS (SRL_FUSED_MAX_BLOCKS / SRL_FUSED_GROUP)
#define SRL_FUSED_CUT_MAX_KPB 64

struct SrlMapSlot {
    unsigned long long key;
    unsigned slab;
    unsigned count;
};
static_assert(sizeof(SrlMapSlot) == 16, "slot must be 16 bytes");

struct SrlSlab {
    float xyz[SRL_CAP][3];
    unsigned count;
    unsigned pad;
    unsigned long long key;
};
static_assert(sizeof(SrlSlab) == SRL_SLAB_BYTES, "slab must be 256 bytes");

struct SrlBlockInfo {
    int accepted;
    unsigned sum_pk;
    int nan_first;
    int num_fallback;
    int planes;
    int pad[3];
};
static_assert(sizeof(SrlBlockInfo) == 32, "block info is 32 bytes");

struct SrlDevOut {
    double HtH[36];
    double Hth[6];
    double loss;
    double d_num_res;
    double d_total_accepted;
    double d_sum_pk;
    double d_nan;
    double d_fallback;
    double d_visited;
    double d_timeout;
    long long last_visited;
    long long pad;
};

struct SrlMailbox {
    SrlDevOut out;
    unsigned long long seq;
    unsigned long long expired;
    unsigned long long pad[10];
    unsigned long long g[2 * (sizeof(SrlDevOut) / 8)];
};
static_assert(sizeof(SrlDevOut) == 52 * 8 && offsetof(SrlDevOut, pad) == 51 * 8, "SrlDevOut is 52 words, the marker word last");
static_assert(offsetof(SrlMailbox, g) % 64 == 0, "the tagged record starts on a cache line");

#define SRL_POSE_BOX_CTRL 42
#define SRL_POSE_BOX_N 43
#define SRL_POSE_BOX_TLAST 44
#define SRL_POSE_BOX_USED 50
#define SRL_POSE_BOX_WRITTEN 56
#define SRL_POSE_BOX_GRANULES 64
#define SRL_ARM_GO 1u
#define SRL_ARM_CANCEL 2u
#define SRL_ARM_EXPIRED 3u
#define SRL_ARM_CODE_MASK 3u
#define SRL_ARM_ALT 4u

#define SRL_REDUCED_DOUBLES 50

#define SRL_MAX_PEERS 8
#define SRL_PEER_ROW 64
#define SRL_PEER_INBOX_GRANULES (2 * SRL_MAX_PEERS * 2 * SRL_PEER_ROW)
#define SRL_PEER_TIMEOUT_MARK 0x9EE9ll
struct SrlPeerTable {
    unsigned long long *inbox[SRL_MAX_PEERS];
    int nranks, rank;
};

struct SrlAssocArgs {
    const double *raw_x, *raw_y, *raw_z;
    const double *aos;
    int n;
    const SrlMapSlot *table;
    unsigned table_mask;
    const unsigned char *slabs;
    int write_rec;
    unsigned inf_off;
    double Rn[9];
    double R[9];
    double t[3];
    double t_last[3];
    double R_il[9];
    double t_il[3];
    double size_voxel;
    double max_dist;
    double lambda_w, lambda_n;
    double power_planarity;
    double nbr_scale;
    int K;
    int min_nb;
    int thr_cap;
    int select_mode;
    int ablate;
    unsigned long long *granules;
    unsigned long long *rec_granules;
    long long cut_max;
    SrlMailbox *mailbox;
    int mail_tagged;
    int pad_mail;
    unsigned long long seq;
    const unsigned long long *pose_box;
    const double *alt_x, *alt_y, *alt_z;
    const double *alt_aos;
    unsigned long long *pose_relay;
    int pose_relayed;
    int pad_relay;
    unsigned pose_epoch;
    unsigned arm_linger_ticks;
    long long *stamps;
    const SrlPeerTable *peer;
    unsigned peer_epoch;
    int peer_slot;
    const float *bound_in;
    float *bound_out;
    int bound_use;
    int pad_bound;
    double *rec;
    unsigned char *status;
    double *partials;
    SrlBlockInfo *binfo;
    int *tap_ids;
    int *tap_ncand;
    double *tap_normal;
    double *tap_a2d;
    double *tap_offset;
};

#define SRL_POSE_DOUBLES 24
static_assert(sizeof(SrlAssocArgs) <= 4096, "the struct travels in the kernarg segment");

struct SrlReduceArgs {
    const double *rec;
    const unsigned char *status;
    const double *partials;
    const SrlBlockInfo *binfo;
    int n;
    int nblocks;
    long long max_res;
    const long long *gather;
    int rank;
    int max_num_residuals;
    SrlDevOut *out;
    SrlMailbox *mailbox;
    unsigned long long seq;
    int kpb;
};

struct SrlSearchArgs {
    const double *q;
    int n;
    const SrlMapSlot *table;
    unsigned table_mask;
    const unsigned char *slabs;
    double size_voxel;
    int K;
    int thr_cap;
    int select_mode;
    int *ids;
    float *nb_xyz;
    int *num_found;
};

hipError_t srl_launch_assoc(const SrlAssocArgs &a, int nb_voxels, int kpw, int wpb, hipStream_t s);
int srl_assoc_lds_bytes(int K, int nb_voxels, int kpw, int wpb);
static inline int srl_keypoints_per_wave(int n) { return n <= 16384 ? 4 : (n <= 32768 ? 8 : 16); }
static inline int srl_keypoints_per_wave_one_round(int n, int num_cu) {
    const int set[7] = {2, 3, 4, 6, 8, 12, 16};
    for (int i = 0; i < 7; ++i) if ((long long)16 * set[i] * num_cu >= n) return set[i];
    return 16;
}
#define SRL_LDS_LIMIT (160 * 1024)
hipError_t srl_launch_reduce(const SrlReduceArgs &a, int mode, hipStream_t s);
hipError_t srl_launch_count(const SrlBlockInfo *binfo, int nblocks, int count_planes, long long *out_total, hipStream_t s);
hipError_t srl_launch_publish(const SrlDevOut *src, SrlMailbox *mb, unsigned long long seq, hipStream_t s);
hipError_t srl_launch_peer_rows(const SrlPeerTable *peer, unsigned epoch, int slot, const SrlDevOut *src, SrlMailbox *mb, unsigned long long seq,
                                const long long *gather_check, hipStream_t s);
hipError_t srl_launch_peer_counts(const SrlPeerTable *peer, unsigned epoch, int slot, const long long *count, long long *gather_out, hipStream_t s);
hipError_t srl_launch_search(const SrlSearchArgs &a, int nb_voxels, hipStream_t s);
struct SrlXform { double R[9], t[3], R_il[9], t_il[3]; };
hipError_t srl_launch_transform(const double *raw_aos, int n, const SrlXform &X, double *out_aos, hipStream_t s);
hipError_t srl_launch_aos_to_soa(const double *aos, int n, double *x, double *y, double *z, hipStream_t s);
hipError_t srl_launch_sqrt(double *io, int n, hipStream_t s);
```

### sr_livo_amd/csrc/srl_kernels.hip

```cpp
#include "srl_device.h"
#include "srl_hash.h"
#include "srl_heap.h"

#include <math.h>
#include <type_traits>

namespace {

struct alignas(8) VoxEnt { unsigned slab; unsigned count; };
struct Surv { double d2; float x, y, z; unsigned id; };
static_assert(sizeof(Surv) == 24, "survivor record is 24 bytes");
static_assert(SRL_SURV_CAP * 24 + (SRL_MAXK + 1) * 8 <= SRL_WAVE_SCRATCH, "general-path scratch (survivors + sorted d2) must fit");
static_assert(64 * 8 + SRL_MAXK * 16 + SRL_MAXK * 4 <= SRL_WAVE_SCRATCH, "heap replay scratch must fit");

__device__ __forceinline__ int lane_id() {
    return __builtin_amdgcn_mbcnt_hi(~0u, __builtin_amdgcn_mbcnt_lo(~0u, 0));
}
__device__ __forceinline__ int lanes_below(unsigned long long m) {
    return __builtin_amdgcn_mbcnt_hi((unsigned)(m >> 32), __builtin_amdgcn_mbcnt_lo((unsigned)m, 0));
}

struct Cand { bool valid; double d2; float x, y, z; unsigned id; };

__device__ __forceinline__ Cand eval_cand(int e, int nv, const VoxEnt *vox, const unsigned char *slabs,
// ... 179 lines not shown
                Surv r; r.d2 = c.d2; r.x = c.x; r.y = c.y; r.z = c.z; r.id = c.id;
                surv[pos] = r;
            }
            c_surv += __popcll(m);
        }
        __builtin_amdgcn_wave_barrier();
        if (c_surv > SRL_SURV_CAP) use_fallback = true;
    }

    if (!use_fallback) {
        const int i = lane;
        const bool act = i < c_surv;
        Surv me;
        if (act) me = surv[i];
        else { me.d2 = __builtin_huge_val(); me.x = me.y = me.z = 0.0f; me.id = 0; }
        int rank = 0;
        for (int j = 0; j < c_surv; ++j) {
            const double dj = surv[j].d2;
            rank += ((dj < me.d2) || (dj == me.d2 && j < i)) ? 1 : 0;
        }
        if (act && rank <= K) sorted[rank] = me.d2;
        __builtin_amdgcn_wave_barrier();
        bool bad = false;
        if (act && rank < K && rank + 1 < c_surv) bad = !(sorted[rank + 1] > me.d2 * SRL_NEAR_TIE);
        tie = __ballot(bad) != 0ull;
        if (!tie && act && rank < K) sink.put(rank, me.x, me.y, me.z, me.id);
        fallback_out = 0;
    } else {
        double last_d2 = -1.0;
        int last_e = -1;
        const int next = total < K + 1 ? total : K + 1;
        for (int r = 0; r < next; ++r) {
            double bd2 = __builtin_huge_val();
            int be = 0x7fffffff;
            for (int j = 0; j < rounds; ++j) {
                const int e = lane + 64 * j;
                const Cand c = eval_cand(e, nv, vox, slabs, qx, qy, qz);
                const bool gt = c.valid && (c.d2 > last_d2 || (c.d2 == last_d2 && e > last_e));
                if (gt && (c.d2 < bd2 || (c.d2 == bd2 && e < be))) { bd2 = c.d2; be = e; }
            }
#pragma unroll
            for (int off = 32; off >= 1; off >>= 1) {
                const double od = __shfl_xor(bd2, off);
                const int oe = __shfl_xor(be, off);
                if (od < bd2 || (od == bd2 && oe < be)) { bd2 = od; be = oe; }
            }
            if (r > 0 && !(bd2 > last_d2 * SRL_NEAR_TIE)) { tie = true; break; }
            if (r < nsel && (be & 63) == lane) {
                const Cand c = eval_cand(be, nv, vox, slabs, qx, qy, qz);
                sink.put(r, c.x, c.y, c.z, c.id);
            }
            last_d2 = bd2;
            last_e = be;
        }
        fallback_out = 1;
    }
    __builtin_amdgcn_wave_barrier();
    if (tie) {
        select_topk_replay(qx, qy, qz, nv, vox, slabs, K, surv, lane, sink, total_out);
        fallback_out = 1;
    }
}

struct LaneRole {
    int pdx, pdy, pdz;
    int c0, slot;
};
__device__ __forceinline__ LaneRole lane_role(int lane) {
    LaneRole r;
    const int pl = lane & 31;
    const int ix = pl / 9, iy = (pl / 3) % 3, iz = pl % 3;
    r.pdx = ix - 1; r.pdy = iy - 1; r.pdz = iz - 1;
    r.c0 = lane / SRL_CAP;
    r.slot = lane - r.c0 * SRL_CAP;
    return r;
}

struct ProbeReq {
    unsigned long long key;
    unsigned h;
    SrlMapSlot s0, s1;
};
__device__ __forceinline__ ProbeReq probe_issue(const int *kv, int kl, const LaneRole &role, const SrlMapSlot *table,
                                                unsigned mask, int lane) {
    ProbeReq r;
    r.key = SRL_EMPTY_KEY; r.h = 0;
    r.s0.key = SRL_EMPTY_KEY; r.s0.slab = 0; r.s0.count = 0;
    r.s1 = r.s0;
    if ((lane & 31) < 27) {
        const int *k = kv + (kl + (lane >> 5)) * 4;
        r.key = srl_pack_key((short)(k[0] + role.pdx), (short)(k[1] + role.pdy), (short)(k[2] + role.pdz));
        r.h = srl_hash_key(r.key) & mask;
        r.s0 = table[r.h];
        r.s1 = table[(r.h + 1) & mask];
    }
    return r;
}
__device__ __forceinline__ int probe_finish(const ProbeReq &r, int thr_cap, const SrlMapSlot *table, unsigned mask,
                                            VoxEnt *vox, int lane, int *ncand_pair, bool cull = false, const float *qf_pair = nullptr,
                                            const int *kv_pair = nullptr, const LaneRole *role = nullptr, float size_voxel = 1.0f) {
    const bool prober = (lane & 31) < 27;
    const bool m0 = prober && r.s0.key == r.key;
    const bool m1 = prober && !m0 && r.s0.key != SRL_EMPTY_KEY && r.s1.key == r.key;
    bool found = m0 || m1;
    unsigned slab = m0 ? r.s0.slab : r.s1.slab, cnt = m0 ? r.s0.count : r.s1.count;
    const bool more = prober && !found && r.s0.key != SRL_EMPTY_KEY && r.s1.key != SRL_EMPTY_KEY;
    if (__ballot(more) != 0ull) {
        if (more) {
            unsigned h = (r.h + 2) & mask;
            for (unsigned probe = 2; probe <= mask; ++probe) {
                const SrlMapSlot sl = table[h];
                if (sl.key == r.key) { slab = sl.slab; cnt = sl.count; found = true; break; }
                if (sl.key == SRL_EMPTY_KEY) break;
                h = (h + 1) & mask;
            }
        }
    }
    found = found && (int)cnt >= thr_cap && cnt > 0;
    {
#if defined(__HIP_DEVICE_COMPILE__)
        int v = found ? (int)cnt : 0;
        v += __builtin_amdgcn_update_dpp(0, v, 0x111, 0xF, 0xF, false);
        v += __builtin_amdgcn_update_dpp(0, v, 0x112, 0xF, 0xF, false);
        v += __builtin_amdgcn_update_dpp(0, v, 0x114, 0xF, 0xF, false);
        v += __builtin_amdgcn_update_dpp(0, v, 0x118, 0xF, 0xF, false);
        v += __builtin_amdgcn_update_dpp(0, v, 0x142, 0xA, 0xF, false);
        if ((lane & 31) == 31) ncand_pair[lane >> 5] = v;
#endif
    }
    if (cull) {
        const int hh = lane >> 5;
        const float *qf = qf_pair + 8 * hh;
        const int *kv = kv_pair + 4 * hh;
        const float r2 = qf[5];
        float bd2 = 0.0f;
        const int pd[3] = {role->pdx, role->pdy, role->pdz};
#pragma unroll
        for (int ax = 0; ax < 3; ++ax) {
            const int v = kv[ax] + pd[ax];
            const float lo = (float)(v > 0 ? v : v - 1) * size_voxel, hi = (float)(v < 0 ? v : v + 1) * size_voxel;
            const float d = fmaxf(fmaxf(lo - qf[ax], qf[ax] - hi), 0.0f);
            bd2 += d * d;
        }
        found = found && bd2 <= r2;
    }
    const unsigned long long m = __ballot(found);
    const unsigned m_lo = (unsigned)m, m_hi = (unsigned)(m >> 32);
    const int nv_a = __popc(m_lo), nv_b = __popc(m_hi);
    if (prober) {
        const bool upper = lane >= 32;
        const unsigned f_lo = found ? m_lo : (~m_lo & 0x7FFFFFFu), f_hi = found ? m_hi : (~m_hi & 0x7FFFFFFu);
        const int below = upper ? (int)__builtin_amdgcn_mbcnt_hi(f_hi, 0u) : (int)__builtin_amdgcn_mbcnt_lo(f_lo, 0u);
        const int nv_own = upper ? nv_b : nv_a;
        VoxEnt ve; ve.slab = found ? slab : 0u; ve.count = found ? cnt : 0u;
        vox[(upper ? 32 : 0) + (found ? below : nv_own + below)] = ve;
    }
    __builtin_amdgcn_wave_barrier();
    return nv_a | (nv_b << 8);
}

struct LdsSink {
    float *col;
    int row;
    int plane;
    int *tap_ids;
    __device__ __forceinline__ void put(int rank, float x, float y, float z, unsigned id) {
        float *p = col + rank * row;
        p[0] = x;
        p[plane] = y;
        p[2 * plane] = z;
        if (tap_ids) tap_ids[rank] = (int)id;
    }
};

struct alignas(16) SurvRec { float x, y, z; int code; };
#define SRL_PAIR_MAX_ROUNDS 4

__device__ __forceinline__ float d2_f32(float px, float py, float pz, float qx, float qy, float qz) {
#pragma clang fp contract(fast)
    const float dx = px - qx, dy = py - qy, dz = pz - qz;
    return dx * dx + dy * dy + dz * dz;
}

template <class Sink>
__device__ __forceinline__ int finish_survivors(double qx, double qy, double qz, int c, const VoxEnt *vox, int K, void *scratch,
                                                int lane, Sink &sink, double *tau_out = nullptr) {
    SurvRec *recs = reinterpret_cast<SurvRec *>(__builtin_assume_aligned(scratch, 16));
    double *keys = reinterpret_cast<double *>(reinterpret_cast<unsigned char *>(scratch) + 1024);
    double *sorted = keys + 66;
    __builtin_amdgcn_wave_barrier();
    const bool act = lane < c;
    SurvRec me;
    me.x = me.y = me.z = 0.0f; me.code = 0;
    double my = __builtin_huge_val();
    if (act) {
        me = recs[lane];
        const double dx = (double)me.x - qx;
        const double dy = (double)me.y - qy;
// ... 21 lines not shown
            const double2 kk = *reinterpret_cast<const double2 *>(keys + j);
            rank += (kk.x < my) ? 1 : 0;
            rank += (kk.y < my) ? 1 : 0;
        }
    }
    const bool win = act && rank < K;
    if (act && rank <= K) sorted[rank] = my;
    __builtin_amdgcn_wave_barrier();
    bool bad = false;
    if (lane >= 1 && lane <= K && lane < c) bad = !(sorted[lane] > sorted[lane - 1] * SRL_NEAR_TIE);
    if (__ballot(bad)) return SEL_TIE;
    if (tau_out && act && rank == K - 1) *tau_out = my;
    if (win) {
        const VoxEnt ve = vox[me.code >> 5];
        sink.put(rank, me.x, me.y, me.z, ve.slab * SRL_CAP + ((unsigned)me.code & 31u));
    }
    __builtin_amdgcn_wave_barrier();
    return SEL_DONE;
}

template <int R>
__device__ __forceinline__ void cand_issue(const VoxEnt *vox, const unsigned char *slabs, unsigned inf_off, const LaneRole &role,
                                           float (&px)[R], float (&py)[R], float (&pz)[R], int &total_out) {
    VoxEnt ve[R];
    const int cbase = role.c0 < 3 ? role.c0 : 0;
#pragma unroll
    for (int j = 0; j < R; ++j) ve[j] = vox[3 * j + cbase];
    const unsigned slot_eff = role.c0 < 3 ? (unsigned)role.slot : 31u;
    const unsigned slot_off = (unsigned)role.slot * 12u;
    unsigned off[R];
    int total = 0;
#pragma unroll
    for (int j = 0; j < R; ++j) {
        const bool h = slot_eff < ve[j].count;
        total += __popcll(__ballot(h));
        off[j] = h ? ve[j].slab * (unsigned)SRL_SLAB_BYTES + slot_off : inf_off;
    }
#pragma unroll
    for (int j = 0; j < R; ++j) {
        const float *p = reinterpret_cast<const float *>(slabs + off[j]);
        px[j] = p[0]; py[j] = p[1]; pz[j] = p[2];
    }
    total_out = total;
}

template <int R>
__device__ __forceinline__ float cand_d2f(const float (&px)[R], const float (&py)[R], const float (&pz)[R], const float *qf, float (&d2f)[R]) {
    const float qxf = qf[0], qyf = qf[1], qzf = qf[2];
    float lmin = __builtin_huge_valf();
#pragma unroll
    for (int j = 0; j < R; ++j) {
        d2f[j] = d2_f32(px[j], py[j], pz[j], qxf, qyf, qzf);
        lmin = fminf(lmin, d2f[j]);
    }
    return lmin;
}
__device__ __forceinline__ float thr_from_bisection(unsigned lo, const float *qf) {
    const float tau_f = __uint_as_float(lo | 0x3FFFFu);
    float thr = 3.4028235e38f;
    if (tau_f < __builtin_huge_valf()) thr = qf[3] + qf[4] * tau_f;
    return thr;
}
template <int R>
__device__ __forceinline__ void cand_compact(const float (&px)[R], const float (&py)[R], const float (&pz)[R], const float (&d2f)[R], float thr,
                                             const unsigned long long (&svm)[R], const LaneRole &role, SurvRec *recs) {
    const int code0 = (role.c0 << 5) | role.slot;
    int base = 0;
    (void)d2f; (void)thr;
#pragma unroll
    for (int j = 0; j < R; ++j) {
        {
            if (__builtin_amdgcn_inverse_ballot_w64(svm[j])) {
                SurvRec r; r.x = px[j]; r.y = py[j]; r.z = pz[j]; r.code = code0 + ((3 * j) << 5);
                recs[base + lanes_below(svm[j])] = r;
            }
            base += __popcll(svm[j]);
        }
    }
}

template <int R, class Sink>
__device__ __forceinline__ int cand_select(const float (&px)[R], const float (&py)[R], const float (&pz)[R], double qx, double qy, double qz,
                                           const float *qf, const VoxEnt *vox, int K, void *scratch, int lane, const LaneRole &role, Sink &sink,
                                           int ablate) {
    float d2f[R];
    const unsigned v = __float_as_uint(cand_d2f<R>(px, py, pz, qf, d2f));
    unsigned lo = 0;
#pragma unroll
    for (int bit = 30; bit >= 18; --bit) {
        const unsigned trial = lo | (1u << bit);
        const int cnt = __popcll(__ballot(v < trial));
        lo = (cnt < K) ? trial : lo;
    }
    const float thr = thr_from_bisection(lo, qf);
    SurvRec *recs = reinterpret_cast<SurvRec *>(__builtin_assume_aligned(scratch, 16));
    unsigned long long svm[R];
    int c = 0;
#pragma unroll
    for (int j = 0; j < R; ++j) {
        svm[j] = __ballot(d2f[j] <= thr);
        c += __popcll(svm[j]);
    }
    if (c > 64) return SEL_OVERFLOW;
    cand_compact<R>(px, py, pz, d2f, thr, svm, role, recs);
    if (ablate & 2) return SEL_DONE;
    return finish_survivors(qx, qy, qz, c, vox, K, scratch, lane, sink, reinterpret_cast<double *>(const_cast<float *>(qf) + 6));
}

template <int R, class Sink>
__device__ __forceinline__ int select_topk_f32_r(double qx, double qy, double qz, const float *qf, int nv, const VoxEnt *vox,
                                                  const unsigned char *slabs, unsigned inf_off, int K, void *scratch, int lane,
                                                  const LaneRole &role, Sink &sink, int &total_out, int ablate) {
    (void)nv;
    float px[R], py[R], pz[R];
    cand_issue<R>(vox, slabs, inf_off, role, px, py, pz, total_out);
    return cand_select<R>(px, py, pz, qx, qy, qz, qf, vox, K, scratch, lane, role, sink, ablate);
}

__device__ __forceinline__ int finish_pair(const double *qa, const double *qb, int ca, int cb, const VoxEnt *vox, int K, void *scratch, int lane,
                                           const LdsSink &sink_a, const LdsSink &sink_b, const float *qfa, const float *qfb) {
    SurvRec *recs = reinterpret_cast<SurvRec *>(__builtin_assume_aligned(scratch, 16));
    double *keys = reinterpret_cast<double *>(reinterpret_cast<unsigned char *>(scratch) + 1024);
    double *sorted = keys + 64;
    __builtin_amdgcn_wave_barrier();
    const int h = lane >> 5, i = lane & 31;
    const int c = h ? cb : ca;
    const bool act = i < c;
    const double *q = h ? qb : qa;
    SurvRec me;
    me.x = me.y = me.z = 0.0f; me.code = 0;
    double my = __builtin_huge_val();
    if (act) {
        me = recs[lane];
        const double dx = (double)me.x - q[0];
        const double dy = (double)me.y - q[1];
        const double dz = (double)me.z - q[2];
        my = (dx * dx + dy * dy) + dz * dz;
    }
    keys[lane] = my;
    sorted[lane] = __builtin_nan("");
    __builtin_amdgcn_wave_barrier();
    const double2 *kp = reinterpret_cast<const double2 *>(keys + 32 * h);
    int rank = 0;
#pragma unroll
    for (int j = 0; j < 16; ++j) {
        const double2 kk = kp[j];
        rank += (kk.x < my) ? 1 : 0;
        rank += (kk.y < my) ? 1 : 0;
    }
    const bool win = act && rank < K;
    if (act && rank <= K) sorted[32 * h + rank] = my;
    __builtin_amdgcn_wave_barrier();
    bool bad = false;
    if (i >= 1 && i <= K && i < c) bad = !(sorted[32 * h + i] > sorted[32 * h + i - 1] * SRL_NEAR_TIE);
    const unsigned long long bm = __ballot(bad);
    const bool tie_a = (unsigned)bm != 0u, tie_b = (unsigned)(bm >> 32) != 0u;
    if (win && !(h ? tie_b : tie_a)) {
        const VoxEnt ve = vox[32 * h + (me.code >> 5)];
        LdsSink s = sink_a;
        if (h) { s.col = sink_b.col; s.tap_ids = sink_b.tap_ids; }
        s.put(rank, me.x, me.y, me.z, ve.slab * SRL_CAP + ((unsigned)me.code & 31u));
        if (rank == K - 1) *reinterpret_cast<double *>(const_cast<float *>(h ? qfb : qfa) + 6) = my;
    }
    __builtin_amdgcn_wave_barrier();
    return (tie_a ? SEL_TIE : SEL_DONE) | ((tie_b ? SEL_TIE : SEL_DONE) << 8);
}

template <int R>
__device__ __forceinline__ int select_pair_f32_r(const double *qa, const double *qb, const float *qfa, const float *qfb, const VoxEnt *vox,
                                                 const unsigned char *slabs, unsigned inf_off, int K, void *scratch, int lane,
                                                 const LaneRole &role, LdsSink &sink_a, LdsSink &sink_b, int &total_a, int &total_b, int ablate) {
    float ax[R], ay[R], az[R], bx[R], by[R], bz[R];
    cand_issue<R>(vox, slabs, inf_off, role, ax, ay, az, total_a);
    cand_issue<R>(vox + 32, slabs, inf_off, role, bx, by, bz, total_b);
    float da[R], db[R];
    const unsigned va = __float_as_uint(cand_d2f<R>(ax, ay, az, qfa, da));
    const unsigned vb = __float_as_uint(cand_d2f<R>(bx, by, bz, qfb, db));
    constexpr unsigned BAND_LO = 0x38000000u, BAND_HI = 0x40000000u, BAND_LAST = 0x3FFC0000u;
    const unsigned ca_v = va < BAND_LO ? BAND_LO : (va > BAND_HI ? BAND_HI : va);
    const unsigned cb_v = vb < BAND_LO ? BAND_LO : (vb > BAND_HI ? BAND_HI : vb);
    unsigned lo_a = BAND_LO, lo_b = BAND_LO;
#pragma unroll
    for (int bit = 26; bit >= 18; --bit) {
        const unsigned ta = lo_a | (1u << bit), tb = lo_b | (1u << bit);
        const int cnt_a = __popcll(__ballot(ca_v < ta));
        const int cnt_b = __popcll(__ballot(cb_v < tb));
        lo_a = (cnt_a < K) ? ta : lo_a;
        lo_b = (cnt_b < K) ? tb : lo_b;
    }
    if (lo_a == BAND_LAST || lo_b == BAND_LAST) {
        lo_a = 0; lo_b = 0;
#pragma nounroll
        for (int bit = 30; bit >= 18; --bit) {
            const unsigned ta = lo_a | (1u << bit), tb = lo_b | (1u << bit);
            const int cnt_a = __popcll(__ballot(va < ta));
            const int cnt_b = __popcll(__ballot(vb < tb));
            lo_a = (cnt_a < K) ? ta : lo_a;
            lo_b = (cnt_b < K) ? tb : lo_b;
        }
    }
    const float thr_a = thr_from_bisection(lo_a, qfa), thr_b = thr_from_bisection(lo_b, qfb);
    unsigned long long sa[R], sb[R];
    int ca = 0, cb = 0;
#pragma unroll
    for (int j = 0; j < R; ++j) {
        sa[j] = __ballot(da[j] <= thr_a);
        sb[j] = __ballot(db[j] <= thr_b);
        ca += __popcll(sa[j]);
        cb += __popcll(sb[j]);
    }
    SurvRec *recs = reinterpret_cast<SurvRec *>(__builtin_assume_aligned(scratch, 16));
    if (ca <= 32 && cb <= 32 && K <= 31 && !(ablate & (2 | 512))) {
        cand_compact<R>(ax, ay, az, da, thr_a, sa, role, recs);
        cand_compact<R>(bx, by, bz, db, thr_b, sb, role, recs + 32);
        return finish_pair(qa, qb, ca, cb, vox, K, scratch, lane, sink_a, sink_b, qfa, qfb);
    }
    int done_a = SEL_OVERFLOW, done_b = SEL_OVERFLOW;
    if (ca <= 64) {
        cand_compact<R>(ax, ay, az, da, thr_a, sa, role, recs);
        done_a = (ablate & 2) ? SEL_DONE : finish_survivors(qa[0], qa[1], qa[2], ca, vox, K, scratch, lane, sink_a, reinterpret_cast<double *>(const_cast<float *>(qfa) + 6));
    }
    __builtin_amdgcn_wave_barrier();
    if (cb <= 64) {
        cand_compact<R>(bx, by, bz, db, thr_b, sb, role, recs);
        done_b = (ablate & 2) ? SEL_DONE : finish_survivors(qb[0], qb[1], qb[2], cb, vox + 32, K, scratch, lane, sink_b, reinterpret_cast<double *>(const_cast<float *>(qfb) + 6));
    }
    return done_a | (done_b << 8);
}

template <class Sink>
__device__ __forceinline__ int select_topk_f32(double qx, double qy, double qz, const float *qf, int nv, const VoxEnt *vox,
                                                const unsigned char *slabs, unsigned inf_off, int K, void *scratch, int lane,
                                                const LaneRole &role, Sink &sink, int &total_out, int ablate) {
    switch ((nv + 2) / 3) {
        case 0: case 1: case 2: case 3:
            return select_topk_f32_r<3>(qx, qy, qz, qf, nv, vox, slabs, inf_off, K, scratch, lane, role, sink, total_out, ablate);
        case 4: return select_topk_f32_r<4>(qx, qy, qz, qf, nv, vox, slabs, inf_off, K, scratch, lane, role, sink, total_out, ablate);
        case 5: return select_topk_f32_r<5>(qx, qy, qz, qf, nv, vox, slabs, inf_off, K, scratch, lane, role, sink, total_out, ablate);
        case 6: return select_topk_f32_r<6>(qx, qy, qz, qf, nv, vox, slabs, inf_off, K, scratch, lane, role, sink, total_out, ablate);
        case 7: return select_topk_f32_r<7>(qx, qy, qz, qf, nv, vox, slabs, inf_off, K, scratch, lane, role, sink, total_out, ablate);
        default: return select_topk_f32_r<9>(qx, qy, qz, qf, nv, vox, slabs, inf_off, K, scratch, lane, role, sink, total_out, ablate);
    }
}

template <class Sink>
__device__ __forceinline__ int select_topk_f32_loop(double qx, double qy, double qz, const float *qf, int nv, const VoxEnt *vox,
                                                    const unsigned char *slabs, unsigned inf_off, int K, void *scratch, int lane,
                                                    const LaneRole &role, Sink &sink, int &total_out) {
    const float kInfF = __builtin_huge_valf();
    const float qxf = qf[0], qyf = qf[1], qzf = qf[2];
    const int rounds = (nv + 2) / 3;
    const int cbase = role.c0 < 3 ? role.c0 : 0;
    const unsigned slot_eff = role.c0 < 3 ? (unsigned)role.slot : 31u;
    const unsigned slot_off = (unsigned)role.slot * 12u;
    float lmin = kInfF;
    int total = 0;
    constexpr int CH = 4;
    auto cand_off = [&](int j, bool &has) {
        const int jj = j < rounds ? j : rounds - 1;
        const VoxEnt ve = vox[3 * jj + cbase];
        has = (j < rounds) && (slot_eff < ve.count);
        return has ? ve.slab * (unsigned)SRL_SLAB_BYTES + slot_off : inf_off;
    };
    for (int j0 = 0; j0 < rounds; j0 += CH) {
        unsigned off[CH];
#pragma unroll
        for (int u = 0; u < CH; ++u) { bool h; off[u] = cand_off(j0 + u, h); total += __popcll(__ballot(h)); }
        float x[CH], y[CH], z[CH];
#pragma unroll
        for (int u = 0; u < CH; ++u) { const float *p = reinterpret_cast<const float *>(slabs + off[u]); x[u] = p[0]; y[u] = p[1]; z[u] = p[2]; }
#pragma unroll
        for (int u = 0; u < CH; ++u) lmin = fminf(lmin, d2_f32(x[u], y[u], z[u], qxf, qyf, qzf));
    }
    total_out = total;
    const unsigned v = __float_as_uint(lmin);
    unsigned lo = 0;
#pragma unroll
    for (int bit = 30; bit >= 18; --bit) {
        const unsigned trial = lo | (1u << bit);
        const int cnt = __popcll(__ballot(v < trial));
        lo = (cnt < K) ? trial : lo;
    }
    const float tau_f = __uint_as_float(lo | 0x3FFFFu);
    float thr = 3.4028235e38f;
    if (tau_f < kInfF) thr = qf[3] + qf[4] * tau_f;

    SurvRec *recs = reinterpret_cast<SurvRec *>(__builtin_assume_aligned(scratch, 16));
    const int code0 = (role.c0 << 5) | role.slot;
    int c = 0;
    for (int j0 = 0; j0 < rounds; j0 += CH) {
        unsigned off[CH];
#pragma unroll
        for (int u = 0; u < CH; ++u) { bool h; off[u] = cand_off(j0 + u, h); }
        float x[CH], y[CH], z[CH];
#pragma unroll
        for (int u = 0; u < CH; ++u) { const float *p = reinterpret_cast<const float *>(slabs + off[u]); x[u] = p[0]; y[u] = p[1]; z[u] = p[2]; }
#pragma unroll
        for (int u = 0; u < CH; ++u) {
            const bool sv = d2_f32(x[u], y[u], z[u], qxf, qyf, qzf) <= thr;
            const unsigned long long m = __ballot(sv);
            if (m != 0ull) {
                const int pos = c + lanes_below(m);
                if (sv && pos < 64) { SurvRec r; r.x = x[u]; r.y = y[u]; r.z = z[u]; r.code = code0 + ((3 * (j0 + u)) << 5); recs[pos] = r; }
                c += __popcll(m);
            }
        }
    }
    if (c > 64) return SEL_OVERFLOW;
    return finish_survivors(qx, qy, qz, c, vox, K, scratch, lane, sink, reinterpret_cast<double *>(const_cast<float *>(qf) + 6));
}

struct D3 { double x, y, z; };
__device__ __forceinline__ D3 d3(double x, double y, double z) { D3 r; r.x = x; r.y = y; r.z = z; return r; }
__device__ __forceinline__ D3 sub(D3 a, D3 b) { return d3(a.x - b.x, a.y - b.y, a.z - b.z); }
__device__ __forceinline__ double dot3(D3 a, D3 b) { return (a.x * b.x + a.y * b.y) + a.z * b.z; }
__device__ __forceinline__ D3 matvec(const double *M, D3 v) {
    return d3((M[0] * v.x + M[1] * v.y) + M[2] * v.z, (M[3] * v.x + M[4] * v.y) + M[5] * v.z,
              (M[6] * v.x + M[7] * v.y) + M[8] * v.z);
}
__device__ __forceinline__ D3 add(D3 a, D3 b) { return d3(a.x + b.x, a.y + b.y, a.z + b.z); }
__device__ __forceinline__ double rcp_nr(double b) {
    double r = __builtin_amdgcn_rcp(b);
    r = __builtin_fma(__builtin_fma(-b, r, 1.0), r, r);
    r = __builtin_fma(__builtin_fma(-b, r, 1.0), r, r);
// ... 232 lines not shown

template <int NB, int FAST, int KPW, int WPB, int DBG = 0, int ARMED = 0>
__device__ __forceinline__ bool assoc_tile(KargBytes karg, const SrlAssocArgs &A, const int tile) {
    constexpr int KPB = WPB * KPW;
    extern __shared__ __attribute__((aligned(16))) unsigned char smem[];
    const int Kn = A.K;
    const int abl = DBG ? A.ablate : 0;
    constexpr bool POSE_LDS = ARMED != 0;
    const LdsLayout L = lds_layout(Kn, NB, KPW, WPB, ARMED);
    const int NB_ROW = L.nb_row;
    const int tid = threadIdx.x;
    const int lane = lane_id();
    const int wave = tid >> 6;
    float *s_nb = reinterpret_cast<float *>(smem + L.off_nb);
    const int nb_plane = Kn * NB_ROW;
    double *s_pw = reinterpret_cast<double *>(smem + L.off_pw);
    double *s_pimu = reinterpret_cast<double *>(smem + L.off_pimu);
    float *s_qf = reinterpret_cast<float *>(smem + L.off_qf);
    int *s_kv = reinterpret_cast<int *>(smem + L.off_kv);
    int *s_nfound = reinterpret_cast<int *>(smem + L.off_nfound);
    int *s_ncand = reinterpret_cast<int *>(smem + L.off_ncand);
    int *s_next = reinterpret_cast<int *>(smem + L.off_next);
    unsigned short *s_defer = reinterpret_cast<unsigned short *>(smem + L.off_defer);
    unsigned char *wbase = smem + L.off_wave + wave * L.wave_bytes;
    VoxEnt *vox = reinterpret_cast<VoxEnt *>(wbase + L.off_vox);
    Surv *surv = reinterpret_cast<Surv *>(wbase + L.off_scratch);
    double *s_wpart = reinterpret_cast<double *>(smem + L.off_wpart);
    int *s_winfo = reinterpret_cast<int *>(smem + L.off_winfo);

    const long long dbg_t0 = (DBG && (abl & 128)) ? (long long)wall_clock64() : 0;
#if defined(__HIP_DEVICE_COMPILE__)
    typedef const __attribute__((address_space(4))) SrlAssocArgs *KernargPtr;
#endif
    double *s_pose = reinterpret_cast<double *>(smem + L.off_pose);
    auto n_pass = [&]() -> int {
        if constexpr (ARMED) return __builtin_amdgcn_readfirstlane(reinterpret_cast<const int *>(s_pose + SRL_POSE_DOUBLES)[1]);
        else return A.n;
    };
    int n_fallback = 0;
#if defined(__HIP_DEVICE_COMPILE__)
    auto tile_stamp = [&](int slot) {
        if constexpr (ARMED) {
            arm_stamp(karg, slot - 8);
        }
    };
#else
    auto tile_stamp = [&](int) {};
#endif
    tile_stamp(10);
    bool use_bounds = A.bound_in != nullptr && A.bound_use > 0;
    if constexpr (ARMED) use_bounds = use_bounds && reinterpret_cast<const int *>(s_pose + SRL_POSE_DOUBLES)[2] == 0 && n_pass() == A.n;
    const int bbase_kp = tile * KPB;
    const int wbase_kp = bbase_kp + wave * KPW;

    if (tid < 4) s_next[tid] = 0;
    if (lane < KPW) {
        const int kq = wave * KPW + lane;
        const int g = wbase_kp + lane;
        D3 p_imu = d3(0, 0, 0), p_w = d3(0, 0, 0);
        if constexpr (ARMED) {
            if (g < n_pass()) {
                p_imu = d3(s_pimu[kq * 3 + 0], s_pimu[kq * 3 + 1], s_pimu[kq * 3 + 2]);
                p_w = add(matvec(s_pose, p_imu), d3(s_pose[18], s_pose[19], s_pose[20]));
            }
        } else {
            if (g < A.n) {
                D3 raw;
                if (A.aos != nullptr) {
                    const double *p = A.aos + 3 * (size_t)g;
                    raw = d3(p[0], p[1], p[2]);
                    const_cast<double *>(A.raw_x)[g] = raw.x; const_cast<double *>(A.raw_y)[g] = raw.y; const_cast<double *>(A.raw_z)[g] = raw.z;
                } else {
                    raw = d3(A.raw_x[g], A.raw_y[g], A.raw_z[g]);
                }
                p_imu = add(matvec(A.R_il, raw), d3(A.t_il[0], A.t_il[1], A.t_il[2]));
                p_w = add(matvec(A.Rn, p_imu), d3(A.t[0], A.t[1], A.t[2]));
            }
            s_pimu[kq * 3 + 0] = p_imu.x; s_pimu[kq * 3 + 1] = p_imu.y; s_pimu[kq * 3 + 2] = p_imu.z;
        }
        s_pw[kq * 3 + 0] = p_w.x; s_pw[kq * 3 + 1] = p_w.y; s_pw[kq * 3 + 2] = p_w.z;
        const bool unit = A.size_voxel == 1.0;
        const int kv[3] = {(int)(short)(int)(unit ? p_w.x : p_w.x / A.size_voxel), (int)(short)(int)(unit ? p_w.y : p_w.y / A.size_voxel),
                           (int)(short)(int)(unit ? p_w.z : p_w.z / A.size_voxel)};
        {
            const float qxf = (float)p_w.x, qyf = (float)p_w.y, qzf = (float)p_w.z;
            const float u = 5.9604645e-8f;
            const float am = fmaxf(fmaxf(fabsf(qxf), fabsf(qyf)), fabsf(qzf)) * u + 1e-30f;
            const float h = 4.0f * am * 0.5001f;
            const float m0 = h * (1.0f + 1e-6f) + 8.0f * u * 1e-6f + 4.0f * am * am;
            const float m1 = 2.0f * h + 16.0f * u;
            float *qf = s_qf + kq * 8;
            qf[0] = qxf; qf[1] = qyf; qf[2] = qzf;
            qf[3] = (2.0f * m0) * 1.00001f;
            qf[4] = (1.0f + 2.0f * m1) * 1.00001f;
            float r2 = __builtin_huge_valf();
            if (use_bounds && g < A.bound_use) {
                const float4 bp = reinterpret_cast<const float4 *>(A.bound_in)[g];
                const float ex = qxf - bp.x, ey = qyf - bp.y, ez = qzf - bp.z;
                const float mag = fmaxf(fabsf(qxf) + fabsf(qyf) + fabsf(qzf), fabsf(bp.x) + fabsf(bp.y) + fabsf(bp.z));
                const float slack = 1e-3f + 1e-6f * mag;
                const float rt = sqrtf(bp.w) * 1.000001f;
                const float sz = (float)A.size_voxel;
                const float bq[3] = {bp.x, bp.y, bp.z};
                bool inside = true;
#pragma unroll
                for (int ax = 0; ax < 3; ++ax) {
                    const int vlo = kv[ax] - NB, vhi = kv[ax] + NB;
                    const float lo = (float)(vlo > 0 ? vlo : vlo - 1) * sz, hi = (float)(vhi < 0 ? vhi : vhi + 1) * sz;
                    inside = inside && (bq[ax] - rt) - slack >= lo && (bq[ax] + rt) + slack <= hi;
                }
                if (inside) {
                    const float r = rt + sqrtf(ex * ex + ey * ey + ez * ez) * 1.000001f + slack;
                    r2 = (r * r) * 1.00001f;
                }
            }
            qf[5] = r2;
            *reinterpret_cast<double *>(qf + 6) = __builtin_huge_val();
        }
        s_kv[kq * 4 + 0] = kv[0];
        s_kv[kq * 4 + 1] = kv[1];
        s_kv[kq * 4 + 2] = kv[2];
        s_nfound[kq] = 0;
        s_ncand[kq] = 0;
    } else if (wave == WPB - 1 && lane < KPW + 2) {
        const int kq = KPB + (lane - KPW);
        s_kv[kq * 4 + 0] = 0; s_kv[kq * 4 + 1] = 0; s_kv[kq * 4 + 2] = 0;
    }
    __syncthreads();
    tile_stamp(11);

    {
        const int left = n_pass() - bbase_kp;
        const int n_here = __builtin_amdgcn_readfirstlane(left < KPB ? left : KPB);
        auto make_sink = [&](int kl) {
            LdsSink sink;
            sink.col = s_nb + kl;
            sink.row = NB_ROW;
            sink.plane = nb_plane;
            sink.tap_ids = A.tap_ids ? (A.tap_ids + (size_t)(bbase_kp + kl) * Kn) : nullptr;
            return sink;
        };
        auto keypoint_general = [&](int kl, bool tie) {
            const double qx = s_pw[kl * 3 + 0], qy = s_pw[kl * 3 + 1], qz = s_pw[kl * 3 + 2];
            LdsSink sink = make_sink(kl);
            int total = 0, fb = 0;
            const int nv = probe_voxels<NB>(qx, qy, qz, A.size_voxel, A.thr_cap, A.table, A.table_mask, vox, lane);
            select_topk(qx, qy, qz, nv, vox, A.slabs, Kn, tie ? 5 : A.select_mode, surv, lane, sink, total, fb);
            n_fallback += (NB == 1) ? 1 : fb;
            if (lane == 0) {
                s_nfound[kl] = total < Kn ? total : Kn;
                s_ncand[kl] = total;
            }
        };
        if constexpr (NB == 1 && FAST != 0) {
            const LaneRole role = lane_role(lane);
            const int npairs = n_here > 0 ? (n_here + 1) >> 1 : 0;
            auto take = [&]() { int p = 0; if (lane == 0) p = atomicAdd(s_next, 1); return __builtin_amdgcn_readfirstlane(p); };
            int cur = take();
            ProbeReq preq;
            if (!(abl & 32)) preq = probe_issue(s_kv, 2 * (cur < npairs ? cur : npairs), role, A.table, A.table_mask, lane);
            while (cur < npairs) {
                const int nxt = take();
                const int nv_pair = __builtin_amdgcn_readfirstlane((abl & 8) ? 0 : probe_finish(preq, A.thr_cap, A.table, A.table_mask, vox, lane, s_ncand + 2 * cur, use_bounds, s_qf + 16 * cur,
                                                                                                               s_kv + 8 * cur, &role, (float)A.size_voxel));
                if (!(abl & 32)) preq = probe_issue(s_kv, 2 * (nxt < npairs ? nxt : npairs), role, A.table, A.table_mask, lane);
                auto file = [&](int kl, int done, int total) {
                    (void)total;
                    if (done == SEL_DONE) {
                    } else {
                        s_defer[atomicAdd(s_next + 1, 1)] = (unsigned short)(kl | (done == SEL_TIE ? 0x8000 : 0));
                    }
                };
                const int r_a = (int)((((unsigned)nv_pair & 0xFFu) + 2u) * 0x5556u >> 16), r_b = (int)(((((unsigned)nv_pair >> 8) & 0xFFu) + 2u) * 0x5556u >> 16);
                const int r_max = r_a > r_b ? r_a : r_b;
                if (2 * cur + 1 < n_here && r_max <= SRL_PAIR_MAX_ROUNDS && !(abl & (4 | 256))) {
                    const int kl = 2 * cur;
                    LdsSink sink_a = make_sink(kl), sink_b = make_sink(kl + 1);
                    int total_a = 0, total_b = 0, done;
                    if (r_max <= 2) done = select_pair_f32_r<2>(s_pw + kl * 3, s_pw + kl * 3 + 3, s_qf + kl * 8, s_qf + kl * 8 + 8, vox, A.slabs, A.inf_off, Kn, surv, lane, role, sink_a, sink_b, total_a, total_b, abl);
                    else if (r_max <= 3) done = select_pair_f32_r<3>(s_pw + kl * 3, s_pw + kl * 3 + 3, s_qf + kl * 8, s_qf + kl * 8 + 8, vox, A.slabs, A.inf_off, Kn, surv, lane, role, sink_a, sink_b, total_a, total_b, abl);
                    else done = select_pair_f32_r<4>(s_pw + kl * 3, s_pw + kl * 3 + 3, s_qf + kl * 8, s_qf + kl * 8 + 8, vox, A.slabs, A.inf_off, Kn, surv, lane, role, sink_a, sink_b, total_a, total_b, abl);
                    (void)total_a; (void)total_b;
                    if (done != (SEL_DONE | (SEL_DONE << 8))) {
                        if (lane == 0) {
                            if ((done & 0xFF) != SEL_DONE) s_defer[atomicAdd(s_next + 1, 1)] = (unsigned short)(kl | ((done & 0xFF) == SEL_TIE ? 0x8000 : 0));
                            if ((done >> 8) != SEL_DONE) s_defer[atomicAdd(s_next + 1, 1)] = (unsigned short)((kl + 1) | ((done >> 8) == SEL_TIE ? 0x8000 : 0));
                        }
                    }
                } else {
#pragma nounroll
                    for (int h = 0; h < 2; ++h) {
                        const int kl = 2 * cur + h;
                        if (kl >= n_here) break;
                        const int nv_fast = h ? (nv_pair >> 8) : (nv_pair & 0xFF);
                        const double qx = s_pw[kl * 3 + 0], qy = s_pw[kl * 3 + 1], qz = s_pw[kl * 3 + 2];
                        LdsSink sink = make_sink(kl);
                        int total = nv_fast;
                        int done = SEL_DONE;
                        if (!(abl & 4)) done = select_topk_f32(qx, qy, qz, s_qf + kl * 8, nv_fast, vox + 32 * h, A.slabs, A.inf_off, Kn, surv, lane, role, sink, total, abl);
                        if (lane == 0) file(kl, done, total);
                    }
                }
                cur = nxt;
            }
        } else if constexpr (NB == 2 && FAST != 0) {
            const LaneRole role = lane_role(lane);
            auto take = [&]() { int p = 0; if (lane == 0) p = atomicAdd(s_next, 1); return __builtin_amdgcn_readfirstlane(p); };
            for (int kl = take(); kl < n_here; kl = take()) {
                const double qx = s_pw[kl * 3 + 0], qy = s_pw[kl * 3 + 1], qz = s_pw[kl * 3 + 2];
                int total_all = 0;
                const int nv = probe_voxels<NB>(qx, qy, qz, A.size_voxel, A.thr_cap, A.table, A.table_mask, vox, lane, use_bounds ? s_qf + kl * 8 : nullptr, &total_all);
                if (lane < 3) { VoxEnt z; z.slab = 0u; z.count = 0u; vox[nv + lane] = z; }
                __builtin_amdgcn_wave_barrier();
                LdsSink sink = make_sink(kl);
                int total = 0;
                const int done = select_topk_f32_loop(qx, qy, qz, s_qf + kl * 8, nv, vox, A.slabs, A.inf_off, Kn, surv, lane, role, sink, total);
                total = total_all;
                if (lane == 0) {
                    if (done == SEL_DONE) {
                        s_nfound[kl] = total < Kn ? total : Kn;
                        s_ncand[kl] = total;
                    } else {
                        s_defer[atomicAdd(s_next + 1, 1)] = (unsigned short)(kl | (done == SEL_TIE ? 0x8000 : 0));
                    }
                }
            }
        } else {
            for (int kl = wave * KPW; kl < (wave + 1) * KPW && kl < n_here; ++kl) keypoint_general(kl, false);
        }
        if constexpr (FAST != 0) {
            __syncthreads();
            const int n_defer = __builtin_amdgcn_readfirstlane(s_next[1]);
            if (n_defer > 0) {
                auto take2 = [&]() { int p = 0; if (lane == 0) p = atomicAdd(s_next + 2, 1); return __builtin_amdgcn_readfirstlane(p); };
                for (int i = take2(); i < n_defer; i = take2()) {
                    const int e = __builtin_amdgcn_readfirstlane((int)s_defer[i]);
                    keypoint_general(e & 0x7FFF, (e & 0x8000) != 0);
                }
            }
        }
    }
    __syncthreads();
    tile_stamp(12);

    if (abl & 64) return true;
#if defined(__HIP_DEVICE_COMPILE__)
    KernargPtr bp = (KernargPtr)karg;
    asm volatile("" : "+s"(bp));
    const __attribute__((address_space(4))) SrlAssocArgs &b = *bp;
#else
    const SrlAssocArgs &b = A;
#endif
    constexpr int LPK = p2_lanes_per_keypoint(KPB);
    constexpr int KP2 = p2_keypoints_per_wave(KPB);
    constexpr int P2W = (KPB + KP2 - 1) / KP2;
    const int w2 = (wave + WPB - (int)(blockIdx.x % WPB)) % WPB;
    const bool p2_wave = w2 < P2W;
    const int klw = lane / LPK, sl = lane % LPK;
    const int kl = (p2_wave ? w2 : 0) * KP2 + klw;
    const bool owner_lane = p2_wave && klw < KP2 && kl < KPB;
    const int n2 = ARMED ? n_pass() : b.n;
    const int g = owner_lane ? bbase_kp + kl : n2;
    auto quad_xor = [](double v, auto ctrl) {
#if defined(__HIP_DEVICE_COMPILE__)
        const long long b = __double_as_longlong(v);
        const int lo = __builtin_amdgcn_update_dpp(0, (int)(unsigned)b, decltype(ctrl)::value, 0xF, 0xF, true);
        const int hi = __builtin_amdgcn_update_dpp(0, (int)(unsigned)((unsigned long long)b >> 32), decltype(ctrl)::value, 0xF, 0xF, true);
        return __longlong_as_double((long long)(((unsigned long long)(unsigned)hi << 32) | (unsigned)lo));
#else
        return v;
#endif
    };
    auto lpk_sum = [&](double v) {
        if (LPK >= 2) v += quad_xor(v, std::integral_constant<int, 0xB1>{});
        if (LPK >= 4) v += quad_xor(v, std::integral_constant<int, 0x4E>{});
        return v;
    };
    int status = 3;
    bool nan_bad = false;
    double J[6] = {0, 0, 0, 0, 0, 0};
    double dist = 0.0, weight = 0.0;
    const int nc2 = owner_lane ? s_ncand[kl] : 0;
// ... 80 lines not shown
        float4 bo;
        bo.x = qf[0]; bo.y = qf[1]; bo.z = qf[2];
        bo.w = (float)tau * 1.0000002f;
        reinterpret_cast<float4 *>(b.bound_out)[g] = bo;
    }
    if (g < n2 && b.write_rec && sl == 0) {
        double2 *r = reinterpret_cast<double2 *>(b.rec + (size_t)g * 8);
        double2 v;
        v.x = J[0]; v.y = J[1]; r[0] = v;
        v.x = J[2]; v.y = J[3]; r[1] = v;
        v.x = J[4]; v.y = J[5]; r[2] = v;
        v.x = dist; v.y = weight; r[3] = v;
        b.status[g] = (unsigned char)status;
        if (b.tap_ncand) b.tap_ncand[g] = s_ncand[kl];
    }

    if (b.rec_granules != nullptr && owner_lane && sl == 0) {
        typedef __attribute__((address_space(1))) unsigned long long gu64r;
        const bool accd = status == 2;
        const double rec8[8] = {J[0], J[1], J[2], J[3], J[4], J[5], dist, weight};
        const unsigned long long tag = (unsigned long long)(unsigned)b.seq << 32;
        gu64r *dst = (gu64r *)(b.rec_granules + ((size_t)blockIdx.x * KPB + kl) * 16);
#pragma unroll
        for (int d = 0; d < 8; ++d) {
            const unsigned long long bits = accd ? (unsigned long long)__double_as_longlong(rec8[d]) : 0ull;
            __hip_atomic_store(dst + 2 * d, tag | (bits & 0xFFFFFFFFull), __ATOMIC_RELAXED, __HIP_MEMORY_SCOPE_AGENT);
            __hip_atomic_store(dst + 2 * d + 1, tag | (bits >> 32), __ATOMIC_RELAXED, __HIP_MEMORY_SCOPE_AGENT);
        }
    }

    if (p2_wave) {
        static_assert(P2W * KP2 * 64 <= WPB * (64 * 8 + SRL_WAVE_SCRATCH), "phase-2 rows must fit in the phase-1 per-wave regions");
        double *s_row = reinterpret_cast<double *>(smem + L.off_wave) + w2 * (KP2 * 8);
        const bool accd = status == 2;
        if (sl == 0 && klw < KP2) {
            const double h = dist * weight;
            double4 v;
            v.x = accd ? J[0] : 0.0; v.y = accd ? J[1] : 0.0; v.z = accd ? J[2] : 0.0; v.w = accd ? J[3] : 0.0;
            *reinterpret_cast<double4 *>(s_row + klw * 8) = v;
            v.x = accd ? J[4] : 0.0; v.y = accd ? J[5] : 0.0; v.z = accd ? h : 0.0; v.w = accd ? dist : 0.0;
            *reinterpret_cast<double4 *>(s_row + klw * 8 + 4) = v;
        }
        __builtin_amdgcn_wave_barrier();
        if (lane < 28) {
            int ia, ib;
            if (lane < 21) {
                int c = lane, r = 0;
                while (c >= 6 - r) { c -= 6 - r; ++r; }
                ia = r; ib = r + c;
            } else if (lane < 27) { ia = lane - 21; ib = 6; }
            else { ia = 7; ib = 7; }
            double acc = 0.0;
#pragma unroll 16
            for (int k = 0; k < KP2; ++k) acc += s_row[k * 8 + ia] * s_row[k * 8 + ib];
            s_wpart[w2 * 32 + lane] = acc;
        }
    }
    if constexpr (ARMED) arm_stamp(karg, 24);
    {
        auto per_keypoint = [](unsigned long long m) {
            if (LPK == 2) {
                m &= 0x5555555555555555ull;
                m = (m | (m >> 1)) & 0x3333333333333333ull;
                m = (m | (m >> 2)) & 0x0F0F0F0F0F0F0F0Full;
                m = (m | (m >> 4)) & 0x00FF00FF00FF00FFull;
                m = (m | (m >> 8)) & 0x0000FFFF0000FFFFull;
                m = (m | (m >> 16)) & 0x00000000FFFFFFFFull;
            } else if (LPK == 4) {
                m &= 0x1111111111111111ull;
                m = (m | (m >> 3)) & 0x0303030303030303ull;
                m = (m | (m >> 6)) & 0x000F000F000F000Full;
                m = (m | (m >> 12)) & 0x000000FF000000FFull;
                m = (m | (m >> 24)) & 0xFFFFull;
            }
            return m;
        };
        const unsigned long long acc_mask = __ballot(status == 2 && sl == 0);
        const unsigned long long nan_mask = __ballot(nan_bad);
        const unsigned long long pln_mask = __ballot((status == 1 || status == 2) && sl == 0);
        int pk = (g < n2 && sl == 0) ? s_ncand[kl] : 0;
#pragma unroll
        for (int off = 32; off >= 1; off >>= 1) pk += __shfl_xor(pk, off);
        if (lane == 0) {
            s_winfo[wave * 8 + 3] = n_fallback;
            if (p2_wave) {
                s_winfo[w2 * 8 + 0] = __popcll(acc_mask);
                s_winfo[w2 * 8 + 1] = pk;
                s_winfo[w2 * 8 + 2] = nan_mask ? 1 + w2 * KP2 + (int)__builtin_ctzll(nan_mask) / LPK : 0;
                s_winfo[w2 * 8 + 4] = __popcll(pln_mask);
                const unsigned long long km = per_keypoint(acc_mask);
                s_winfo[w2 * 8 + 5] = (int)(unsigned)km;
                s_winfo[w2 * 8 + 6] = (int)(unsigned)(km >> 32);
            }
        }
    }
    __syncthreads();
    tile_stamp(13);

    if (DBG && (b.ablate & 128) && (tid == 28 || tid == 29 || tid == 30))
        b.partials[(size_t)blockIdx.x * SRL_PART_STRIDE + tid] =
            (tid == 28) ? (double)dbg_t0 : ((tid == 29) ? (double)(long long)wall_clock64() : (double)__builtin_amdgcn_s_getreg(6164) );
    if (tid < 28 && b.granules == nullptr) {
        double v = s_wpart[tid];
#pragma unroll
        for (int w = 1; w < P2W; ++w) v += s_wpart[w * 32 + tid];
        b.partials[(size_t)blockIdx.x * SRL_PART_STRIDE + tid] = v;
    }
    if (tid == 0) {
        SrlBlockInfo bi;
        bi.accepted = 0; bi.sum_pk = 0; bi.nan_first = 0; bi.num_fallback = 0; bi.planes = 0;
        bi.pad[0] = bi.pad[1] = bi.pad[2] = 0;
        for (int w = 0; w < WPB; ++w) bi.num_fallback += s_winfo[w * 8 + 3];
        for (int w = 0; w < P2W; ++w) {
            bi.accepted += s_winfo[w * 8 + 0]; bi.sum_pk += (unsigned)s_winfo[w * 8 + 1];
            if (bi.nan_first == 0) bi.nan_first = s_winfo[w * 8 + 2];
            bi.planes += s_winfo[w * 8 + 4];
        }
        b.binfo[blockIdx.x] = bi;
    }
    return b.granules == nullptr;
}

template <class Take>
__device__ __forceinline__ bool peer_exchange(const SrlPeerTable *pt, unsigned epoch, int slot, int lane, int nwords,
                                              unsigned long long mine, Take take) {
    typedef __attribute__((address_space(1))) unsigned long long gu64;
    const int G = pt->nranks, me = pt->rank;
    const bool act = lane < nwords;
    const unsigned long long tag = (unsigned long long)epoch << 32;
    const size_t slot_off = (size_t)slot * SRL_MAX_PEERS * (2 * SRL_PEER_ROW);
    if (act) {
        const unsigned long long lo = tag | (unsigned)mine, hi = tag | (unsigned)(mine >> 32);
        for (int r = 0; r < G; ++r) {
            unsigned long long *dst = pt->inbox[r] + slot_off + (size_t)me * (2 * SRL_PEER_ROW);
            __hip_atomic_store((gu64 *)(dst + lane), lo, __ATOMIC_RELAXED, __HIP_MEMORY_SCOPE_SYSTEM);
            __hip_atomic_store((gu64 *)(dst + SRL_PEER_ROW + lane), hi, __ATOMIC_RELAXED, __HIP_MEMORY_SCOPE_SYSTEM);
        }
    }
    bool ok = true;
    const unsigned long long *own = pt->inbox[me] + slot_off;
    for (int r = 0; r < G; ++r) {
        if (act) {
            const unsigned long long *src = own + (size_t)r * (2 * SRL_PEER_ROW);
            unsigned long long x0, x1;
            unsigned spins = 0;
            for (;;) {
                x0 = __hip_atomic_load((gu64 *)(src + lane), __ATOMIC_RELAXED, __HIP_MEMORY_SCOPE_SYSTEM);
                x1 = __hip_atomic_load((gu64 *)(src + SRL_PEER_ROW + lane), __ATOMIC_RELAXED, __HIP_MEMORY_SCOPE_SYSTEM);
                if ((unsigned)(x0 >> 32) == epoch && (unsigned)(x1 >> 32) == epoch) break;
                if (++spins > (1u << 20)) { ok = false; x0 = x1 = 0ull; break; }
                __builtin_amdgcn_s_sleep(8);
            }
            take(r, (x1 << 32) | (unsigned long long)(unsigned)x0);
        }
    }
    return __ballot(!ok) == 0ull;
}

template <int KPW, int WPB>
__device__ __forceinline__ void finish_rows(KargBytes karg, const unsigned epoch, const int n_total) {
#if defined(__HIP_DEVICE_COMPILE__)
    constexpr int KPB = WPB * KPW;
    extern __shared__ __attribute__((aligned(16))) unsigned char smem[];
    typedef const __attribute__((address_space(4))) SrlAssocArgs *KernargPtr;
    typedef __attribute__((address_space(1))) unsigned long long gu64;
    KernargPtr bq = (KernargPtr)karg;
    asm volatile("" : "+s"(bq));
    const __attribute__((address_space(4))) SrlAssocArgs &b = *bq;
    const int tid = threadIdx.x;
    const int lane = lane_id();
    const int wave = tid >> 6;
    (void)lane; (void)wave;
    auto put_f = [](double *p, double x) { *p = x; };
    auto put_i = [](long long *p, long long x) { *p = x; };
    auto mail_out = [&](const SrlDevOut *staged) {
        constexpr int NW = (int)(sizeof(SrlDevOut) / 8);
        if (tid < 64) {
            __builtin_amdgcn_fence(__ATOMIC_RELEASE, "wavefront"); __builtin_amdgcn_wave_barrier(); __builtin_amdgcn_fence(__ATOMIC_ACQUIRE, "wavefront");
            const unsigned long long w = tid < NW ? reinterpret_cast<const unsigned long long *>(staged)[tid] : 0ull;
            if (b.mail_tagged) {
                if (tid < NW) store_granule_pair(&b.mailbox->g[2 * tid], (unsigned)b.seq, w);
            } else {
                if (tid < NW) __hip_atomic_store(reinterpret_cast<unsigned long long *>(&b.mailbox->out) + tid, w, __ATOMIC_RELAXED, __HIP_MEMORY_SCOPE_SYSTEM);
                asm volatile("s_waitcnt vmcnt(0)" ::: "memory");
                if (tid == 0) __hip_atomic_store(&b.mailbox->seq, b.seq, __ATOMIC_RELEASE, __HIP_MEMORY_SCOPE_SYSTEM);
            }
        }
    };
    if (b.cut_max > 0) {
        if constexpr (KPB <= SRL_FUSED_CUT_MAX_KPB && WPB == 16) {
            constexpr int NT = 64 * WPB, NPART = NT / 32, INF = 8;
            __syncthreads();
            double *s_part = reinterpret_cast<double *>(smem);
            double *s_recd = reinterpret_cast<double *>(smem + NPART * 32 * 8);
            long long *s_wacc = reinterpret_cast<long long *>(smem + NPART * 32 * 8 + SRL_FUSED_CUT_MAX_KPB * 64);
// ... 848 lines not shown
```

Baseline: 10790 sweeps/s.

## Reuse previous-iteration voxel rows and distance bound to skip probes and bisection

Each keypoint's 27 neighbour-voxel lookups (slab and count) are cached in a per-keypoint row buffer, tagged with the voxel key. On the next ESIKF iteration the hash probe is skipped when the key still matches. A second path seeds the top-K candidate threshold from the previous iteration's distance bound, and falls back to the full bit bisection only when more than 32 candidates survive. Both are enabled by default (bits=3). The cost is extra global writes of 128 bytes per keypoint per pass, plus added branching and register pressure in the probe and select code.

Result: slower. 10190 sweeps/s (-5.5%).

```diff
diff --git a/include/srlivo_hip_debug.h b/include/srlivo_hip_debug.h
--- a/include/srlivo_hip_debug.h
+++ b/include/srlivo_hip_debug.h
@@ -21,6 +21,8 @@
 int srl_debug_set_ablate(srl_ctx *ctx, int bits);
 int srl_debug_set_fused_reduce(srl_ctx *ctx, int enable);
 int srl_debug_set_bound_culling(srl_ctx *ctx, int enable);
+int srl_debug_set_bound_reuse(srl_ctx *ctx, int bits);
+int srl_debug_bound_reuse_counts(srl_ctx *ctx, long long *rows_used, long long *bisect_skipped);
 int srl_debug_set_pose_box(srl_ctx *ctx, int kind);
 int srl_debug_set_arm_linger(srl_ctx *ctx, double host_linger_us, double kernel_linger_us);
 int srl_debug_pass_stamps(srl_ctx *ctx, int enable, long long *gpu_out, long long *host_out);
diff --git a/sr_livo_amd/capi.py b/sr_livo_amd/capi.py
--- a/sr_livo_amd/capi.py
+++ b/sr_livo_amd/capi.py
@@ -225,6 +225,8 @@
         "srl_debug_set_ablate": ([p, C.c_int], C.c_int),
         "srl_debug_set_fused_reduce": ([p, C.c_int], C.c_int),
         "srl_debug_set_bound_culling": ([p, C.c_int], C.c_int),
+        "srl_debug_set_bound_reuse": ([p, C.c_int], C.c_int),
+        "srl_debug_bound_reuse_counts": ([p, C.POINTER(C.c_longlong), C.POINTER(C.c_longlong)], C.c_int),
         "srl_debug_set_pose_box": ([p, C.c_int], C.c_int),
         "srl_debug_set_arm_linger": ([p, C.c_double, C.c_double], C.c_int),
         "srl_debug_pass_stamps": ([p, C.c_int, p, p], C.c_int),
@@ -730,6 +732,14 @@
     def set_bound_culling(self, on):
         self._chk(self.lib.srl_debug_set_bound_culling(self.h, 1 if on else 0), "srl_debug_set_bound_culling")
 
+    def set_bound_reuse(self, bits):
+        self._chk(self.lib.srl_debug_set_bound_reuse(self.h, int(bits)), "srl_debug_set_bound_reuse")
+
+    def bound_reuse_counts(self):
+        a, b = C.c_longlong(0), C.c_longlong(0)
+        self._chk(self.lib.srl_debug_bound_reuse_counts(self.h, C.byref(a), C.byref(b)), "srl_debug_bound_reuse_counts")
+        return int(a.value), int(b.value)
+
     def set_search_select_mode(self, mode):
         self._chk(self.lib.srl_debug_set_search_select_mode(self.h, int(mode)), "srl_debug_set_search_select_mode")
 
diff --git a/sr_livo_amd/csrc/srl_capi.cpp b/sr_livo_amd/csrc/srl_capi.cpp
--- a/sr_livo_amd/csrc/srl_capi.cpp
+++ b/sr_livo_amd/csrc/srl_capi.cpp
@@ -44,7 +44,9 @@
     if ((rc = ensure(ctx, ctx->d_rec, (size_t)cap * 8))) return rc;
     if ((rc = ensure(ctx, ctx->d_status, (size_t)cap))) return rc;
     if ((rc = ensure(ctx, ctx->d_bound, (size_t)cap * 4))) return rc;
+    if ((rc = ensure(ctx, ctx->d_nrow, (size_t)cap * 32))) return rc;
     ctx->bound_n = 0;
+    ctx->row_n = 0;
     if ((rc = ensure(ctx, ctx->d_partials, (size_t)nblocks * SRL_PART_STRIDE))) return rc;
     if ((rc = ensure(ctx, ctx->d_binfo, (size_t)nblocks))) return rc;
     ctx->work_cap = cap;
@@ -177,7 +179,7 @@
     if (ctx->d_sub_kept) hipFree(ctx->d_sub_kept);
     if (ctx->d_sub_seen) hipFree(ctx->d_sub_seen);
     void *bufs[] = {ctx->d_corr_in, ctx->d_corr_rel, ctx->d_corr_imu, ctx->d_corr_raw, ctx->d_corr_seg, ctx->d_frame_raw, ctx->d_frame_world, ctx->d_table, ctx->d_slabs, ctx->d_raw, ctx->d_rec, ctx->d_status, ctx->d_partials, ctx->d_binfo,
-                    ctx->d_out, ctx->d_count, ctx->d_bound, ctx->d_granules, ctx->d_rec_granules, ctx->d_raw_next, ctx->d_stage_next, ctx->d_stage_cur, ctx->d_tap_ids, ctx->d_tap_ncand, ctx->d_tap_normal, ctx->d_tap_a2d,
+                    ctx->d_out, ctx->d_count, ctx->d_bound, ctx->d_nrow, ctx->d_granules, ctx->d_rec_granules, ctx->d_raw_next, ctx->d_stage_next, ctx->d_stage_cur, ctx->d_tap_ids, ctx->d_tap_ncand, ctx->d_tap_normal, ctx->d_tap_a2d,
                     ctx->d_tap_offset, ctx->d_gather, ctx->d_peer, ctx->d_mail};
     for (int r = 0; r < SRL_MAX_PEERS; r++) if (ctx->peer_mapped[r]) hipIpcCloseMemHandle(ctx->peer_mapped[r]);
     if (ctx->d_inbox) hipFree(ctx->d_inbox);
@@ -911,6 +913,11 @@
         a.bound_out = ctx->d_bound;
         a.bound_in = ctx->bound_mode != 0 ? ctx->d_bound : nullptr;
         a.bound_use = a.bound_in ? std::min(ctx->bound_n, n_eff) : 0;
+        a.bound_reuse = a.bound_in ? ctx->bound_reuse : 0;
+        const bool fast = ctx->select_mode == 0 || ctx->select_mode == 4;
+        const bool rows = (a.bound_reuse & 1) != 0 && p.nb == 1 && fast && ctx->ablate == 0;
+        a.row_out = rows ? ctx->d_nrow : nullptr;
+        a.row_in = rows && a.bound_use > 0 && ctx->row_n >= a.bound_use ? ctx->d_nrow : nullptr;
     }
     if (p.fused) {
         a.granules = ctx->d_granules;
@@ -970,6 +977,7 @@
     sg.pose_box = nullptr; sg.pose_relay = nullptr; sg.pose_relayed = 0; sg.pose_epoch = 0; sg.arm_linger_ticks = 0;
     sg.raw_x = sg.raw_y = sg.raw_z = nullptr; sg.alt_x = sg.alt_y = sg.alt_z = nullptr; sg.n = 0; sg.aos = nullptr; sg.alt_aos = nullptr;
     sg.bound_use = 0;
+    sg.row_in = nullptr;
     return sg;
 }
 
@@ -1054,6 +1062,7 @@
     SrlAssocArgs nx = a;
     nx.seq = ctx->seq + 1;
     nx.bound_use = a.bound_in ? a.n : 0;
+    nx.row_in = a.bound_in ? a.row_out : nullptr;
     const bool has_alt = ctx->d_raw_next != nullptr && ctx->next_cap > 0 && ctx->d_stage_next != nullptr;
     nx.aos = nullptr;
     nx.alt_aos = has_alt ? ctx->d_stage_next : nullptr;
@@ -1234,6 +1243,7 @@
 
     if (a.aos != nullptr && n_eff > ctx->soa_valid_n) ctx->soa_valid_n = n_eff;
     ctx->bound_n = n_eff;
+    ctx->row_n = a.row_out != nullptr ? n_eff : 0;
     ctx->last_K = p.K;
     ctx->last_nb = p.nb;
     ctx->last_visited_local = last_visited_local;
@@ -1453,6 +1463,25 @@
     SRL_DISARM(ctx);
     ctx->bound_mode = enable ? 1 : 0;
     ctx->bound_n = 0;
+    return SRL_OK;
+}
+int srl_debug_set_bound_reuse(srl_ctx *ctx, int bits) {
+    if (!ctx || bits < 0 || bits > 3) return SRL_ERR_BAD_ARG;
+    SRL_DISARM(ctx);
+    ctx->bound_reuse = bits;
+    ctx->bound_n = 0;
+    return SRL_OK;
+}
+int srl_debug_bound_reuse_counts(srl_ctx *ctx, long long *rows_used, long long *bisect_skipped) {
+    if (!ctx || !rows_used || !bisect_skipped) return SRL_ERR_BAD_ARG;
+    *rows_used = 0; *bisect_skipped = 0;
+    SRL_DISARM(ctx);
+    const int nb = ctx->last_nblocks;
+    if (nb <= 0 || !ctx->d_binfo) return SRL_OK;
+    std::vector<SrlBlockInfo> bi((size_t)nb);
+    HIPCHK(ctx, hipStreamSynchronize(ctx->stream));
+    HIPCHK(ctx, hipMemcpy(bi.data(), ctx->d_binfo, (size_t)nb * sizeof(SrlBlockInfo), hipMemcpyDeviceToHost));
+    for (const SrlBlockInfo &b : bi) { *rows_used += b.rows_used; *bisect_skipped += b.bisect_skipped; }
     return SRL_OK;
 }
 int srl_debug_set_fused_reduce(srl_ctx *ctx, int enable) {
diff --git a/sr_livo_amd/csrc/srl_ctx.h b/sr_livo_amd/csrc/srl_ctx.h
--- a/sr_livo_amd/csrc/srl_ctx.h
+++ b/sr_livo_amd/csrc/srl_ctx.h
@@ -65,6 +65,9 @@
     int bound_n = 0;
     int bound_sig[4] = {0, 0, 0, 0};
     int bound_mode = 1;
+    unsigned *d_nrow = nullptr;
+    int row_n = 0;
+    int bound_reuse = 3;
     bool tail_pending = false;
     int cur_slot = 0, cur_prefix_n = 0;
 
diff --git a/sr_livo_amd/csrc/srl_device.h b/sr_livo_amd/csrc/srl_device.h
--- a/sr_livo_amd/csrc/srl_device.h
+++ b/sr_livo_amd/csrc/srl_device.h
@@ -47,7 +47,9 @@
     int nan_first;
     int num_fallback;
     int planes;
-    int pad[3];
+    int rows_used;
+    int bisect_skipped;
+    int pad;
 };
 static_assert(sizeof(SrlBlockInfo) == 32, "block info is 32 bytes");
 
@@ -146,7 +148,9 @@
     const float *bound_in;
     float *bound_out;
     int bound_use;
-    int pad_bound;
+    int bound_reuse;
+    const unsigned *row_in;
+    unsigned *row_out;
     double *rec;
     unsigned char *status;
     double *partials;
diff --git a/sr_livo_amd/csrc/srl_kernels.hip b/sr_livo_amd/csrc/srl_kernels.hip
--- a/sr_livo_amd/csrc/srl_kernels.hip
+++ b/sr_livo_amd/csrc/srl_kernels.hip
@@ -285,23 +285,36 @@
     SrlMapSlot s0, s1;
 };
 __device__ __forceinline__ ProbeReq probe_issue(const int *kv, int kl, const LaneRole &role, const SrlMapSlot *table,
-                                                unsigned mask, int lane) {
+                                                unsigned mask, int lane, const unsigned *rows = nullptr) {
     ProbeReq r;
     r.key = SRL_EMPTY_KEY; r.h = 0;
     r.s0.key = SRL_EMPTY_KEY; r.s0.slab = 0; r.s0.count = 0;
     r.s1 = r.s0;
-    if ((lane & 31) < 27) {
-        const int *k = kv + (kl + (lane >> 5)) * 4;
-        r.key = srl_pack_key((short)(k[0] + role.pdx), (short)(k[1] + role.pdy), (short)(k[2] + role.pdz));
-        r.h = srl_hash_key(r.key) & mask;
-        r.s0 = table[r.h];
-        r.s1 = table[(r.h + 1) & mask];
+    const bool prober = (lane & 31) < 27;
+    const int *k = kv + (kl + (lane >> 5)) * 4;
+    const bool cached = rows != nullptr && (k[3] & 1) != 0;
+    const bool probes = prober && !cached;
+    if (__ballot(probes) != 0ull) {
+        if (probes) {
+            r.key = srl_pack_key((short)(k[0] + role.pdx), (short)(k[1] + role.pdy), (short)(k[2] + role.pdz));
+            r.h = srl_hash_key(r.key) & mask;
+            r.s0 = table[r.h];
+            r.s1 = table[(r.h + 1) & mask];
+        }
+    }
+    if (rows != nullptr) {
+        if (prober && cached) {
+            const unsigned e = rows[(kl + (lane >> 5)) * 32 + (lane & 31)];
+            r.key = 0ull; r.s0.key = 0ull;
+            r.s0.slab = e >> 5; r.s0.count = e & 31u;
+        }
     }
     return r;
 }
 __device__ __forceinline__ int probe_finish(const ProbeReq &r, int thr_cap, const SrlMapSlot *table, unsigned mask,
                                             VoxEnt *vox, int lane, int *ncand_pair, bool cull = false, const float *qf_pair = nullptr,
-                                            const int *kv_pair = nullptr, const LaneRole *role = nullptr, float size_voxel = 1.0f) {
+                                            const int *kv_pair = nullptr, const LaneRole *role = nullptr, float size_voxel = 1.0f,
+                                            unsigned *row_pair = nullptr, int row_halves = 0) {
     const bool prober = (lane & 31) < 27;
     const bool m0 = prober && r.s0.key == r.key;
     const bool m1 = prober && !m0 && r.s0.key != SRL_EMPTY_KEY && r.s1.key == r.key;
@@ -317,6 +330,15 @@
                 if (sl.key == SRL_EMPTY_KEY) break;
                 h = (h + 1) & mask;
             }
+        }
+    }
+    if (row_pair != nullptr) {
+        const int hh = lane >> 5, pl = lane & 31;
+        const int *kvh = kv_pair + 4 * hh;
+        if (hh < row_halves && (kvh[3] & 1) == 0 && pl != 27 && pl != 31) {
+            unsigned w = (found && prober) ? ((slab << 5) | cnt) : 0u;
+            if (pl >= 28) w = (unsigned)kvh[pl - 28];
+            row_pair[hh * 32 + pl] = w;
         }
     }
     found = found && (int)cnt >= thr_cap && cnt > 0;
@@ -504,24 +526,38 @@
 template <int R, class Sink>
 __device__ __forceinline__ int cand_select(const float (&px)[R], const float (&py)[R], const float (&pz)[R], double qx, double qy, double qz,
                                            const float *qf, const VoxEnt *vox, int K, void *scratch, int lane, const LaneRole &role, Sink &sink,
-                                           int ablate) {
+                                           int ablate, int from_bound = 0) {
     float d2f[R];
     const unsigned v = __float_as_uint(cand_d2f<R>(px, py, pz, qf, d2f));
-    unsigned lo = 0;
-#pragma unroll
-    for (int bit = 30; bit >= 18; --bit) {
-        const unsigned trial = lo | (1u << bit);
-        const int cnt = __popcll(__ballot(v < trial));
-        lo = (cnt < K) ? trial : lo;
-    }
-    const float thr = thr_from_bisection(lo, qf);
     SurvRec *recs = reinterpret_cast<SurvRec *>(__builtin_assume_aligned(scratch, 16));
     unsigned long long svm[R];
+    float thr = 0.0f;
     int c = 0;
-#pragma unroll
-    for (int j = 0; j < R; ++j) {
-        svm[j] = __ballot(d2f[j] <= thr);
-        c += __popcll(svm[j]);
+    bool have = false;
+    if (from_bound) {
+        thr = qf[3] + qf[4] * qf[5];
+#pragma unroll
+        for (int j = 0; j < R; ++j) {
+            svm[j] = __ballot(d2f[j] <= thr);
+            c += __popcll(svm[j]);
+        }
+        have = c <= 32;
+    }
+    if (!have) {
+        unsigned lo = 0;
+#pragma unroll
+        for (int bit = 30; bit >= 18; --bit) {
+            const unsigned trial = lo | (1u << bit);
+            const int cnt = __popcll(__ballot(v < trial));
+            lo = (cnt < K) ? trial : lo;
+        }
+        thr = thr_from_bisection(lo, qf);
+        c = 0;
+#pragma unroll
+        for (int j = 0; j < R; ++j) {
+            svm[j] = __ballot(d2f[j] <= thr);
+            c += __popcll(svm[j]);
+        }
     }
     if (c > 64) return SEL_OVERFLOW;
     cand_compact<R>(px, py, pz, d2f, thr, svm, role, recs);
@@ -532,11 +568,11 @@
 template <int R, class Sink>
 __device__ __forceinline__ int select_topk_f32_r(double qx, double qy, double qz, const float *qf, int nv, const VoxEnt *vox,
                                                   const unsigned char *slabs, unsigned inf_off, int K, void *scratch, int lane,
-                                                  const LaneRole &role, Sink &sink, int &total_out, int ablate) {
+                                                  const LaneRole &role, Sink &sink, int &total_out, int ablate, int from_bound = 0) {
     (void)nv;
     float px[R], py[R], pz[R];
     cand_issue<R>(vox, slabs, inf_off, role, px, py, pz, total_out);
-    return cand_select<R>(px, py, pz, qx, qy, qz, qf, vox, K, scratch, lane, role, sink, ablate);
+    return cand_select<R>(px, py, pz, qx, qy, qz, qf, vox, K, scratch, lane, role, sink, ablate, from_bound);
 }
 
 __device__ __forceinline__ int finish_pair(const double *qa, const double *qb, int ca, int cb, const VoxEnt *vox, int K, void *scratch, int lane,
@@ -591,45 +627,64 @@
 template <int R>
 __device__ __forceinline__ int select_pair_f32_r(const double *qa, const double *qb, const float *qfa, const float *qfb, const VoxEnt *vox,
                                                  const unsigned char *slabs, unsigned inf_off, int K, void *scratch, int lane,
-                                                 const LaneRole &role, LdsSink &sink_a, LdsSink &sink_b, int &total_a, int &total_b, int ablate) {
+                                                 const LaneRole &role, LdsSink &sink_a, LdsSink &sink_b, int &total_a, int &total_b, int ablate,
+                                                 const int *kv_pair, int &n_count) {
     float ax[R], ay[R], az[R], bx[R], by[R], bz[R];
     cand_issue<R>(vox, slabs, inf_off, role, ax, ay, az, total_a);
     cand_issue<R>(vox + 32, slabs, inf_off, role, bx, by, bz, total_b);
     float da[R], db[R];
     const unsigned va = __float_as_uint(cand_d2f<R>(ax, ay, az, qfa, da));
     const unsigned vb = __float_as_uint(cand_d2f<R>(bx, by, bz, qfb, db));
-    constexpr unsigned BAND_LO = 0x38000000u, BAND_HI = 0x40000000u, BAND_LAST = 0x3FFC0000u;
-    const unsigned ca_v = va < BAND_LO ? BAND_LO : (va > BAND_HI ? BAND_HI : va);
-    const unsigned cb_v = vb < BAND_LO ? BAND_LO : (vb > BAND_HI ? BAND_HI : vb);
-    unsigned lo_a = BAND_LO, lo_b = BAND_LO;
-#pragma unroll
-    for (int bit = 26; bit >= 18; --bit) {
-        const unsigned ta = lo_a | (1u << bit), tb = lo_b | (1u << bit);
-        const int cnt_a = __popcll(__ballot(ca_v < ta));
-        const int cnt_b = __popcll(__ballot(cb_v < tb));
-        lo_a = (cnt_a < K) ? ta : lo_a;
-        lo_b = (cnt_b < K) ? tb : lo_b;
-    }
-    if (lo_a == BAND_LAST || lo_b == BAND_LAST) {
-        lo_a = 0; lo_b = 0;
-#pragma nounroll
-        for (int bit = 30; bit >= 18; --bit) {
+    float thr_a = 0.0f, thr_b = 0.0f;
+    unsigned long long sa[R], sb[R];
+    int ca = 0, cb = 0;
+    bool from_bound = false;
+    if (__builtin_amdgcn_readfirstlane(kv_pair[3] & kv_pair[7] & 2) != 0) {
+        thr_a = qfa[3] + qfa[4] * qfa[5];
+        thr_b = qfb[3] + qfb[4] * qfb[5];
+#pragma unroll
+        for (int j = 0; j < R; ++j) {
+            sa[j] = __ballot(da[j] <= thr_a);
+            sb[j] = __ballot(db[j] <= thr_b);
+            ca += __popcll(sa[j]);
+            cb += __popcll(sb[j]);
+        }
+        from_bound = ca <= 32 && cb <= 32;
+        n_count += from_bound ? 0x10000 : 0;
+    }
+    if (!from_bound) {
+        constexpr unsigned BAND_LO = 0x38000000u, BAND_HI = 0x40000000u, BAND_LAST = 0x3FFC0000u;
+        const unsigned ca_v = va < BAND_LO ? BAND_LO : (va > BAND_HI ? BAND_HI : va);
+        const unsigned cb_v = vb < BAND_LO ? BAND_LO : (vb > BAND_HI ? BAND_HI : vb);
+        unsigned lo_a = BAND_LO, lo_b = BAND_LO;
+#pragma unroll
+        for (int bit = 26; bit >= 18; --bit) {
             const unsigned ta = lo_a | (1u << bit), tb = lo_b | (1u << bit);
-            const int cnt_a = __popcll(__ballot(va < ta));
-            const int cnt_b = __popcll(__ballot(vb < tb));
+            const int cnt_a = __popcll(__ballot(ca_v < ta));
+            const int cnt_b = __popcll(__ballot(cb_v < tb));
             lo_a = (cnt_a < K) ? ta : lo_a;
             lo_b = (cnt_b < K) ? tb : lo_b;
         }
-    }
-    const float thr_a = thr_from_bisection(lo_a, qfa), thr_b = thr_from_bisection(lo_b, qfb);
-    unsigned long long sa[R], sb[R];
-    int ca = 0, cb = 0;
-#pragma unroll
-    for (int j = 0; j < R; ++j) {
-        sa[j] = __ballot(da[j] <= thr_a);
-        sb[j] = __ballot(db[j] <= thr_b);
-        ca += __popcll(sa[j]);
-        cb += __popcll(sb[j]);
+        if (lo_a == BAND_LAST || lo_b == BAND_LAST) {
+            lo_a = 0; lo_b = 0;
+#pragma nounroll
+            for (int bit = 30; bit >= 18; --bit) {
+                const unsigned ta = lo_a | (1u << bit), tb = lo_b | (1u << bit);
+                const int cnt_a = __popcll(__ballot(va < ta));
+                const int cnt_b = __popcll(__ballot(vb < tb));
+                lo_a = (cnt_a < K) ? ta : lo_a;
+                lo_b = (cnt_b < K) ? tb : lo_b;
+            }
+        }
+        thr_a = thr_from_bisection(lo_a, qfa); thr_b = thr_from_bisection(lo_b, qfb);
+        ca = 0; cb = 0;
+#pragma unroll
+        for (int j = 0; j < R; ++j) {
+            sa[j] = __ballot(da[j] <= thr_a);
+            sb[j] = __ballot(db[j] <= thr_b);
+            ca += __popcll(sa[j]);
+            cb += __popcll(sb[j]);
+        }
     }
     SurvRec *recs = reinterpret_cast<SurvRec *>(__builtin_assume_aligned(scratch, 16));
     if (ca <= 32 && cb <= 32 && K <= 31 && !(ablate & (2 | 512))) {
@@ -653,15 +708,15 @@
 template <class Sink>
 __device__ __forceinline__ int select_topk_f32(double qx, double qy, double qz, const float *qf, int nv, const VoxEnt *vox,
                                                 const unsigned char *slabs, unsigned inf_off, int K, void *scratch, int lane,
-                                                const LaneRole &role, Sink &sink, int &total_out, int ablate) {
+                                                const LaneRole &role, Sink &sink, int &total_out, int ablate, int from_bound = 0) {
     switch ((nv + 2) / 3) {
         case 0: case 1: case 2: case 3:
-            return select_topk_f32_r<3>(qx, qy, qz, qf, nv, vox, slabs, inf_off, K, scratch, lane, role, sink, total_out, ablate);
-        case 4: return select_topk_f32_r<4>(qx, qy, qz, qf, nv, vox, slabs, inf_off, K, scratch, lane, role, sink, total_out, ablate);
-        case 5: return select_topk_f32_r<5>(qx, qy, qz, qf, nv, vox, slabs, inf_off, K, scratch, lane, role, sink, total_out, ablate);
-        case 6: return select_topk_f32_r<6>(qx, qy, qz, qf, nv, vox, slabs, inf_off, K, scratch, lane, role, sink, total_out, ablate);
-        case 7: return select_topk_f32_r<7>(qx, qy, qz, qf, nv, vox, slabs, inf_off, K, scratch, lane, role, sink, total_out, ablate);
-        default: return select_topk_f32_r<9>(qx, qy, qz, qf, nv, vox, slabs, inf_off, K, scratch, lane, role, sink, total_out, ablate);
+            return select_topk_f32_r<3>(qx, qy, qz, qf, nv, vox, slabs, inf_off, K, scratch, lane, role, sink, total_out, ablate, from_bound);
+        case 4: return select_topk_f32_r<4>(qx, qy, qz, qf, nv, vox, slabs, inf_off, K, scratch, lane, role, sink, total_out, ablate, from_bound);
+        case 5: return select_topk_f32_r<5>(qx, qy, qz, qf, nv, vox, slabs, inf_off, K, scratch, lane, role, sink, total_out, ablate, from_bound);
+        case 6: return select_topk_f32_r<6>(qx, qy, qz, qf, nv, vox, slabs, inf_off, K, scratch, lane, role, sink, total_out, ablate, from_bound);
+        case 7: return select_topk_f32_r<7>(qx, qy, qz, qf, nv, vox, slabs, inf_off, K, scratch, lane, role, sink, total_out, ablate, from_bound);
+        default: return select_topk_f32_r<9>(qx, qy, qz, qf, nv, vox, slabs, inf_off, K, scratch, lane, role, sink, total_out, ablate, from_bound);
     }
 }
 
@@ -1060,6 +1115,7 @@
         const bool unit = A.size_voxel == 1.0;
         const int kv[3] = {(int)(short)(int)(unit ? p_w.x : p_w.x / A.size_voxel), (int)(short)(int)(unit ? p_w.y : p_w.y / A.size_voxel),
                            (int)(short)(int)(unit ? p_w.z : p_w.z / A.size_voxel)};
+        int kflags = 0;
         {
             const float qxf = (float)p_w.x, qyf = (float)p_w.y, qzf = (float)p_w.z;
             const float u = 5.9604645e-8f;
@@ -1074,6 +1130,12 @@
             float r2 = __builtin_huge_valf();
             if (use_bounds && g < A.bound_use) {
                 const float4 bp = reinterpret_cast<const float4 *>(A.bound_in)[g];
+                if constexpr (NB == 1 && FAST != 0) {
+                    if (A.row_in != nullptr && (A.bound_reuse & 1)) {
+                        const int4 tag = *reinterpret_cast<const int4 *>(A.row_in + (size_t)g * 32 + 28);
+                        kflags = (tag.x == kv[0] && tag.y == kv[1] && tag.z == kv[2]) ? 1 : 0;
+                    }
+                }
                 const float ex = qxf - bp.x, ey = qyf - bp.y, ez = qzf - bp.z;
                 const float mag = fmaxf(fabsf(qxf) + fabsf(qyf) + fabsf(qzf), fabsf(bp.x) + fabsf(bp.y) + fabsf(bp.z));
                 const float slack = 1e-3f + 1e-6f * mag;
@@ -1094,15 +1156,21 @@
             }
             qf[5] = r2;
             *reinterpret_cast<double *>(qf + 6) = __builtin_huge_val();
+            if (r2 < __builtin_huge_valf() && (A.bound_reuse & 2)) kflags |= 2;
         }
         s_kv[kq * 4 + 0] = kv[0];
         s_kv[kq * 4 + 1] = kv[1];
         s_kv[kq * 4 + 2] = kv[2];
+        s_kv[kq * 4 + 3] = kflags;
+        {
+            const int nrows = __popcll(__ballot((kflags & 1) != 0));
+            if (lane == 0) s_winfo[wave * 8 + 7] = nrows;
+        }
         s_nfound[kq] = 0;
         s_ncand[kq] = 0;
     } else if (wave == WPB - 1 && lane < KPW + 2) {
         const int kq = KPB + (lane - KPW);
-        s_kv[kq * 4 + 0] = 0; s_kv[kq * 4 + 1] = 0; s_kv[kq * 4 + 2] = 0;
+        s_kv[kq * 4 + 0] = 0; s_kv[kq * 4 + 1] = 0; s_kv[kq * 4 + 2] = 0; s_kv[kq * 4 + 3] = 0;
     }
     __syncthreads();
     tile_stamp(11);
@@ -1134,14 +1202,26 @@
             const LaneRole role = lane_role(lane);
             const int npairs = n_here > 0 ? (n_here + 1) >> 1 : 0;
             auto take = [&]() { int p = 0; if (lane == 0) p = atomicAdd(s_next, 1); return __builtin_amdgcn_readfirstlane(p); };
+            auto rows_now = [&]() -> unsigned * {
+#if defined(__HIP_DEVICE_COMPILE__)
+                KernargPtr q = (KernargPtr)karg;
+                asm volatile("" : "+s"(q));
+                unsigned *r = q->row_out;
+#else
+                unsigned *r = A.row_out;
+#endif
+                return r != nullptr ? r + (size_t)bbase_kp * 32 : nullptr;
+            };
             int cur = take();
             ProbeReq preq;
-            if (!(abl & 32)) preq = probe_issue(s_kv, 2 * (cur < npairs ? cur : npairs), role, A.table, A.table_mask, lane);
+            if (!(abl & 32)) preq = probe_issue(s_kv, 2 * (cur < npairs ? cur : npairs), role, A.table, A.table_mask, lane, rows_now());
             while (cur < npairs) {
                 const int nxt = take();
+                unsigned *const rows = rows_now();
                 const int nv_pair = __builtin_amdgcn_readfirstlane((abl & 8) ? 0 : probe_finish(preq, A.thr_cap, A.table, A.table_mask, vox, lane, s_ncand + 2 * cur, use_bounds, s_qf + 16 * cur,
-                                                                                                               s_kv + 8 * cur, &role, (float)A.size_voxel));
-                if (!(abl & 32)) preq = probe_issue(s_kv, 2 * (nxt < npairs ? nxt : npairs), role, A.table, A.table_mask, lane);
+                                                                                                               s_kv + 8 * cur, &role, (float)A.size_voxel,
+                                                                                                               rows ? rows + 64 * cur : nullptr, n_here - 2 * cur));
+                if (!(abl & 32)) preq = probe_issue(s_kv, 2 * (nxt < npairs ? nxt : npairs), role, A.table, A.table_mask, lane, rows_now());
                 auto file = [&](int kl, int done, int total) {
                     (void)total;
                     if (done == SEL_DONE) {
@@ -1155,9 +1235,9 @@
                     const int kl = 2 * cur;
                     LdsSink sink_a = make_sink(kl), sink_b = make_sink(kl + 1);
                     int total_a = 0, total_b = 0, done;
-                    if (r_max <= 2) done = select_pair_f32_r<2>(s_pw + kl * 3, s_pw + kl * 3 + 3, s_qf + kl * 8, s_qf + kl * 8 + 8, vox, A.slabs, A.inf_off, Kn, surv, lane, role, sink_a, sink_b, total_a, total_b, abl);
-                    else if (r_max <= 3) done = select_pair_f32_r<3>(s_pw + kl * 3, s_pw + kl * 3 + 3, s_qf + kl * 8, s_qf + kl * 8 + 8, vox, A.slabs, A.inf_off, Kn, surv, lane, role, sink_a, sink_b, total_a, total_b, abl);
-                    else done = select_pair_f32_r<4>(s_pw + kl * 3, s_pw + kl * 3 + 3, s_qf + kl * 8, s_qf + kl * 8 + 8, vox, A.slabs, A.inf_off, Kn, surv, lane, role, sink_a, sink_b, total_a, total_b, abl);
+                    if (r_max <= 2) done = select_pair_f32_r<2>(s_pw + kl * 3, s_pw + kl * 3 + 3, s_qf + kl * 8, s_qf + kl * 8 + 8, vox, A.slabs, A.inf_off, Kn, surv, lane, role, sink_a, sink_b, total_a, total_b, abl, s_kv + kl * 4, n_fallback);
+                    else if (r_max <= 3) done = select_pair_f32_r<3>(s_pw + kl * 3, s_pw + kl * 3 + 3, s_qf + kl * 8, s_qf + kl * 8 + 8, vox, A.slabs, A.inf_off, Kn, surv, lane, role, sink_a, sink_b, total_a, total_b, abl, s_kv + kl * 4, n_fallback);
+                    else done = select_pair_f32_r<4>(s_pw + kl * 3, s_pw + kl * 3 + 3, s_qf + kl * 8, s_qf + kl * 8 + 8, vox, A.slabs, A.inf_off, Kn, surv, lane, role, sink_a, sink_b, total_a, total_b, abl, s_kv + kl * 4, n_fallback);
                     (void)total_a; (void)total_b;
                     if (done != (SEL_DONE | (SEL_DONE << 8))) {
                         if (lane == 0) {
@@ -1175,7 +1255,8 @@
                         LdsSink sink = make_sink(kl);
                         int total = nv_fast;
                         int done = SEL_DONE;
-                        if (!(abl & 4)) done = select_topk_f32(qx, qy, qz, s_qf + kl * 8, nv_fast, vox + 32 * h, A.slabs, A.inf_off, Kn, surv, lane, role, sink, total, abl);
+                        if (!(abl & 4)) done = select_topk_f32(qx, qy, qz, s_qf + kl * 8, nv_fast, vox + 32 * h, A.slabs, A.inf_off, Kn, surv, lane, role, sink, total, abl,
+                                                               __builtin_amdgcn_readfirstlane(s_kv[kl * 4 + 3] & 2));
                         if (lane == 0) file(kl, done, total);
                     }
                 }
@@ -1422,7 +1503,8 @@
 #pragma unroll
         for (int off = 32; off >= 1; off >>= 1) pk += __shfl_xor(pk, off);
         if (lane == 0) {
-            s_winfo[wave * 8 + 3] = n_fallback;
+            s_winfo[wave * 8 + 3] = n_fallback & 0xFFFF;
+            s_winfo[wave * 8 + 7] += (n_fallback >> 16) << 8;
             if (p2_wave) {
                 s_winfo[w2 * 8 + 0] = __popcll(acc_mask);
                 s_winfo[w2 * 8 + 1] = pk;
@@ -1449,8 +1531,8 @@
     if (tid == 0) {
         SrlBlockInfo bi;
         bi.accepted = 0; bi.sum_pk = 0; bi.nan_first = 0; bi.num_fallback = 0; bi.planes = 0;
-        bi.pad[0] = bi.pad[1] = bi.pad[2] = 0;
-        for (int w = 0; w < WPB; ++w) bi.num_fallback += s_winfo[w * 8 + 3];
+        bi.rows_used = 0; bi.bisect_skipped = 0; bi.pad = 0;
+        for (int w = 0; w < WPB; ++w) { bi.num_fallback += s_winfo[w * 8 + 3]; bi.rows_used += s_winfo[w * 8 + 7] & 0xFF; bi.bisect_skipped += s_winfo[w * 8 + 7] >> 8; }
         for (int w = 0; w < P2W; ++w) {
             bi.accepted += s_winfo[w * 8 + 0]; bi.sum_pk += (unsigned)s_winfo[w * 8 + 1];
             if (bi.nan_first == 0) bi.nan_first = s_winfo[w * 8 + 2];
```
